# jhbastek/PhysicsInformedDiffusionModels

Hardware: AMD Instinct MI355X
Metric: training samples/sec (UNet+PDE-residual step), 64x64 Darcy (higher is better)
Workload: dtype f32

## Files before the change

### physicsinformeddiffusionmodels_amd/csrc/k_attn_proj.hip

```cpp
#include "pidm_launch.h"

namespace pidm {

static const int kLapDH = 32;
constexpr int kLapSmallNT = 1024;
static const int kLapTileLd = 33;

__device__ __forceinline__ float lap_exp(float x) { return __expf(x); }
__device__ __forceinline__ int lap_row(int r, int half) { return (r & 3) + 8 * (r >> 2) + 4 * half; }

static int lap_nper_div() {
  const char* e = knob("PIDM_LAP_NPER_DIV");
  const int v = e ? atoi(e) : 1;
  return (v == 2 || v == 4) ? v : 1;
}
static int lap_nper(int N, int C, int slabs) {
  int n = (slabs == 1 ? 512 : 256) * 32 / C;
  if (slabs == 3) n = (C == 32) ? 32 : n / 2;
  if (slabs == 2 && n / lap_nper_div() >= 64) n /= lap_nper_div();
  while (n > 32 && N % n) n >>= 1;
  return n;
}

template <int CB>
__global__ void __launch_bounds__(512) lap_kctx_kernel(const float* __restrict__ xn, const float* __restrict__ wqkv,
                                                       float* __restrict__ part, int N, int heads, int nper) {
  constexpr int C = 32 * CB, CP = C + 4;
  HIP_DYNAMIC_SHARED(float, smem)
  float* xs = smem;
  float* fs = smem + (size_t)nper * CP;
  const int tid = threadIdx.x, lane = tid & 63, half = lane >> 5, l31 = lane & 31;
  const int wave = __builtin_amdgcn_readfirstlane(tid >> 6);
  const int NS = N / nper;
  const int b = blockIdx.x / NS, ns = blockIdx.x % NS;
  const int HD = heads * kLapDH;
  const float* xb = xn + ((size_t)b * N + (size_t)ns * nper) * C;
  for (int e = tid; e < nper * (C / 4); e += 512) {
    const int px = e / (C / 4), q = e - px * (C / 4);
    *reinterpret_cast<f32x4*>(xs + (size_t)px * CP + 4 * q) = *reinterpret_cast<const f32x4*>(xb + (size_t)px * C + 4 * q);
  }
  __syncthreads();
  const int h = wave;
  if (h >= heads) return;
  f32x4 wk[C / 8];
  const float* wrow = wqkv + ((size_t)HD + h * kLapDH + l31) * C + 4 * half;
#pragma unroll
  for (int g8 = 0; g8 < C / 8; ++g8) wk[g8] = *reinterpret_cast<const f32x4*>(wrow + 8 * g8);
  f32x16 M[CB];
#pragma unroll
  for (int cb = 0; cb < CB; ++cb)
    for (int r = 0; r < 16; ++r) M[cb][r] = 0.f;
  float mrun = -3.0e38f, zp = 0.f;
  float* fw = fs + wave * 32;
  for (int t = 0; t < nper / 32; ++t) {
    f32x16 kt;
    for (int r = 0; r < 16; ++r) kt[r] = 0.f;
    const float* arow = xs + (size_t)(t * 32 + l31) * CP + 4 * half;
#pragma unroll
    for (int g8 = 0; g8 < C / 8; ++g8) {
      const f32x4 a4 = *reinterpret_cast<const f32x4*>(arow + 8 * g8);
#pragma unroll
      for (int s = 0; s < 4; ++s) kt = __builtin_amdgcn_mfma_f32_32x32x2f32(a4[s], wk[g8][s], kt, 0, 0, 0);
    }
    float tm = kt[0];
#pragma unroll
    for (int r = 1; r < 16; ++r) tm = fmaxf(tm, kt[r]);
    tm = fmaxf(tm, pidm_other_half(tm));
    if (__any(tm > mrun)) {
      const float mn = fmaxf(mrun, tm);
      const float f = lap_exp(mrun - mn);
      zp *= f;
      mrun = mn;
      if (half == 0) fw[l31] = f;
      PIDM_WAVE_LDS_SYNC();
#pragma unroll
      for (int q4 = 0; q4 < 4; ++q4) {
        const f32x4 f4 = *reinterpret_cast<const f32x4*>(fw + 8 * q4 + 4 * half);
#pragma unroll
        for (int cb = 0; cb < CB; ++cb)
#pragma unroll
          for (int i = 0; i < 4; ++i) M[cb][4 * q4 + i] *= f4[i];
      }
      PIDM_WAVE_LDS_SYNC();
    }
#pragma unroll
    for (int r = 0; r < 16; ++r) {
      kt[r] = lap_exp(kt[r] - mrun);
      zp += kt[r];
    }
#pragma unroll
    for (int r = 0; r < 16; ++r) {
      const float* brow = xs + (size_t)(t * 32 + lap_row(r, half)) * CP + l31;
#pragma unroll
      for (int cb = 0; cb < CB; ++cb) M[cb] = __builtin_amdgcn_mfma_f32_32x32x2f32(kt[r], brow[32 * cb], M[cb], 0, 0, 0);
    }
  }
  const float z = zp + pidm_other_half(zp);
  float* o = part + ((size_t)blockIdx.x * heads + h) * (size_t)(32 * C + 64);
#pragma unroll
  for (int cb = 0; cb < CB; ++cb)
#pragma unroll
    for (int r = 0; r < 16; ++r) o[(size_t)lap_row(r, half) * C + 32 * cb + l31] = M[cb][r];
  if (half == 0) {
    o[32 * C + l31] = mrun;
    o[32 * C + 32 + l31] = z;
  }
}

static int lap_nper_split(int N, int C) {
  int n = 256 * 32 / C;
  if (n / lap_nper_div() >= 64) n /= lap_nper_div();
  while (n > 32 && N % n) n >>= 1;
  return n;
}
static int lap_groups(int heads, int ntiles) {
  const char* e = knob("PIDM_LAP_GROUPS");
  int g = 8 / heads;
  if (e && atoi(e) > 0 && atoi(e) < g) g = atoi(e);
  while (g > 1 && ntiles % g) --g;
  return g < 1 ? 1 : g;
}
template <int CB>
__global__ void __launch_bounds__(512) lap_kctx_split_kernel(const float* __restrict__ xn, const float* __restrict__ wqkv,
                                                             float* __restrict__ part, int N, int heads, int nper) {
  constexpr int C = 32 * CB, RA = 6 * C + 16;
  HIP_DYNAMIC_SHARED(float, smemf)
  char* smem = reinterpret_cast<char*>(smemf);
  const int RT = nper * 2 + 16;
  char* XA = smem;
  char* XT = smem + (size_t)nper * RA;
  float* fs = reinterpret_cast<float*>(XT + (size_t)3 * C * RT);
  const int tid = threadIdx.x, lane = tid & 63, half = lane >> 5, l31 = lane & 31;
  const int wave = __builtin_amdgcn_readfirstlane(tid >> 6);
  const int NS = N / nper;
  const int b = blockIdx.x / NS, ns = blockIdx.x % NS;
  const int HD = heads * kLapDH;
  const float* xb = xn + ((size_t)b * N + (size_t)ns * nper) * C;
  {
    constexpr int QN = C / 4, GP = 16 / QN;
    const int q = lane & (QN - 1), pb = (lane & 15) / QN, la = lane >> 4;
    for (int sl = wave; sl < nper / (4 * GP); sl += 8) {
      const int px = (sl * GP + pb) * 4 + la;
      const f32x4 v = *reinterpret_cast<const f32x4*>(xb + (size_t)px * C + 4 * q);
      typedef unsigned u32x2_t __attribute__((ext_vector_type(2)));
      unsigned a0, a1, a2, b0, b1, b2;
      pidm_split3_pk(v[0], v[1], a0, a1, a2);
      pidm_split3_pk(v[2], v[3], b0, b1, b2);
      char* da = XA + (size_t)px * RA + 8 * q;
      *reinterpret_cast<u32x2_t*>(da) = u32x2_t{a0, b0};
      *reinterpret_cast<u32x2_t*>(da + 2 * C) = u32x2_t{a1, b1};
      *reinterpret_cast<u32x2_t*>(da + 4 * C) = u32x2_t{a2, b2};
      unsigned t0 = __float_as_uint(v[0]), t1 = __float_as_uint(v[1]), t2 = __float_as_uint(v[2]), t3 = __float_as_uint(v[3]);
      {
        const auto s02 = __builtin_amdgcn_permlane32_swap(t0, t2, false, false);
        const auto s13 = __builtin_amdgcn_permlane32_swap(t1, t3, false, false);
        const auto s01 = __builtin_amdgcn_permlane16_swap(s02[0], s13[0], false, false);
        const auto s23 = __builtin_amdgcn_permlane16_swap(s02[1], s13[1], false, false);
        t0 = s01[0]; t1 = s01[1]; t2 = s23[0]; t3 = s23[1];
      }
      pidm_split3_pk(__uint_as_float(t0), __uint_as_float(t1), a0, a1, a2);
      pidm_split3_pk(__uint_as_float(t2), __uint_as_float(t3), b0, b1, b2);
      char* dt = XT + (size_t)(4 * q + la) * RT + (size_t)((sl * GP + pb) * 4) * 2;
      *reinterpret_cast<u32x2_t*>(dt) = u32x2_t{a0, b0};
      *reinterpret_cast<u32x2_t*>(dt + (size_t)C * RT) = u32x2_t{a1, b1};
      *reinterpret_cast<u32x2_t*>(dt + (size_t)2 * C * RT) = u32x2_t{a2, b2};
    }
  }
  __syncthreads();
  const int h = wave;
  if (h >= heads) return;
  u32x4 wk[C / 16][3];
  {
    const float* wrow = wqkv + ((size_t)HD + h * kLapDH + l31) * C + 8 * half;
#pragma unroll
    for (int s = 0; s < C / 16; ++s) {
      const f32x4 w0 = *reinterpret_cast<const f32x4*>(wrow + 16 * s), w1 = *reinterpret_cast<const f32x4*>(wrow + 16 * s + 4);
      unsigned p0[4], p1[4], p2[4];
      pidm_split3_pk(w0[0], w0[1], p0[0], p1[0], p2[0]);
      pidm_split3_pk(w0[2], w0[3], p0[1], p1[1], p2[1]);
      pidm_split3_pk(w1[0], w1[1], p0[2], p1[2], p2[2]);
      pidm_split3_pk(w1[2], w1[3], p0[3], p1[3], p2[3]);
      wk[s][0] = u32x4{p0[0], p0[1], p0[2], p0[3]};
      wk[s][1] = u32x4{p1[0], p1[1], p1[2], p1[3]};
      wk[s][2] = u32x4{p2[0], p2[1], p2[2], p2[3]};
    }
  }
  f32x16 M[CB];
#pragma unroll
  for (int cb = 0; cb < CB; ++cb)
    for (int r = 0; r < 16; ++r) M[cb][r] = 0.f;
  float mrun = -3.0e38f, zp = 0.f;
  float* fw = fs + wave * 32;
#define PIDM_LAP_SIX(acc_, a_, b_)                                                                                 \
  acc_ = pidm_mfma_bf16_32x32x16(a_[2], b_[0], acc_);                                                              \
  acc_ = pidm_mfma_bf16_32x32x16(a_[0], b_[2], acc_);                                                              \
  acc_ = pidm_mfma_bf16_32x32x16(a_[1], b_[1], acc_);                                                              \
  acc_ = pidm_mfma_bf16_32x32x16(a_[1], b_[0], acc_);                                                              \
  acc_ = pidm_mfma_bf16_32x32x16(a_[0], b_[1], acc_);                                                              \
  acc_ = pidm_mfma_bf16_32x32x16(a_[0], b_[0], acc_);
  for (int t = 0; t < nper / 32; ++t) {
    f32x16 kt;
    for (int r = 0; r < 16; ++r) kt[r] = 0.f;
    const char* arow = XA + (size_t)(t * 32 + l31) * RA + 16 * half;
#pragma unroll
    for (int s = 0; s < C / 16; ++s) {
      u32x4 xa[3];
#pragma unroll
      for (int pc = 0; pc < 3; ++pc) xa[pc] = *reinterpret_cast<const u32x4*>(arow + pc * 2 * C + 32 * s);
      PIDM_LAP_SIX(kt, xa, wk[s])
    }
    float tm = kt[0];
#pragma unroll
    for (int r = 1; r < 16; ++r) tm = fmaxf(tm, kt[r]);
    tm = fmaxf(tm, pidm_other_half(tm));
    if (__any(tm > mrun)) {
      const float mn = fmaxf(mrun, tm);
      const float f = lap_exp(mrun - mn);
      zp *= f;
      mrun = mn;
      if (half == 0) fw[l31] = f;
      PIDM_WAVE_LDS_SYNC();
#pragma unroll
      for (int q4 = 0; q4 < 4; ++q4) {
        const f32x4 f4 = *reinterpret_cast<const f32x4*>(fw + 8 * q4 + 4 * half);
#pragma unroll
        for (int cb = 0; cb < CB; ++cb)
#pragma unroll
          for (int i = 0; i < 4; ++i) M[cb][4 * q4 + i] *= f4[i];
      }
      PIDM_WAVE_LDS_SYNC();
    }
#pragma unroll
    for (int r = 0; r < 16; ++r) {
      kt[r] = lap_exp(kt[r] - mrun);
      zp += kt[r];
    }
#pragma unroll
    for (int s = 0; s < 2; ++s) {
      u32x4 ea[3];
      {
        unsigned p0[4], p1[4], p2[4];
#pragma unroll
        for (int j = 0; j < 4; ++j) pidm_split3_pk(kt[8 * s + 2 * j], kt[8 * s + 2 * j + 1], p0[j], p1[j], p2[j]);
        ea[0] = u32x4{p0[0], p0[1], p0[2], p0[3]};
        ea[1] = u32x4{p1[0], p1[1], p1[2], p1[3]};
        ea[2] = u32x4{p2[0], p2[1], p2[2], p2[3]};
      }
#pragma unroll
      for (int cb = 0; cb < CB; ++cb) {
        u32x4 xb4[3];
        const char* brow = XT + (size_t)(32 * cb + l31) * RT + (size_t)(t * 32 + 16 * s + 4 * half) * 2;
#pragma unroll
        for (int pc = 0; pc < 3; ++pc) {
          typedef unsigned u32x2_t __attribute__((ext_vector_type(2)));
          const u32x2_t lo = *reinterpret_cast<const u32x2_t*>(brow + (size_t)pc * C * RT);
          const u32x2_t hi = *reinterpret_cast<const u32x2_t*>(brow + (size_t)pc * C * RT + 16);
          xb4[pc] = u32x4{lo[0], lo[1], hi[0], hi[1]};
        }
        PIDM_LAP_SIX(M[cb], ea, xb4)
      }
    }
  }
#undef PIDM_LAP_SIX
  const float z = zp + pidm_other_half(zp);
  float* o = part + ((size_t)blockIdx.x * heads + h) * (size_t)(32 * C + 64);
#pragma unroll
  for (int cb = 0; cb < CB; ++cb)
#pragma unroll
    for (int r = 0; r < 16; ++r) o[(size_t)lap_row(r, half) * C + 32 * cb + l31] = M[cb][r];
  if (half == 0) {
    o[32 * C + l31] = mrun;
    o[32 * C + 32 + l31] = z;
  }
}

__global__ void __launch_bounds__(kLapSmallNT) lap_kctx_final_kernel(const float* __restrict__ part, const float* __restrict__ wqkv,
                                                             const float* __restrict__ wout, float* __restrict__ kst,
                                                             float* __restrict__ Mmat, float* __restrict__ ctx,
                                                             float* __restrict__ P, int N, int heads, int C, int NS) {
  HIP_DYNAMIC_SHARED(float, smem)
  float* sM = smem;
  float* sW = sM + 32 * C;
  float* sC = sW + 32 * (C + 1) + C;
  float* sw = sC + 32 * 33;
  float* sst = sw + NS * 32;
  __shared__ float sm_[32], siz[32];
  constexpr int NT = kLapSmallNT;
  const int b = blockIdx.x / heads, h = blockIdx.x % heads, tid = threadIdx.x;
  const int HD = heads * kLapDH;
  const size_t pstride = (size_t)(32 * C + 64);
  const float* p0 = part + ((size_t)b * NS * heads + h) * pstride;
  for (int e = tid; e < NS * 64; e += NT) sst[e] = p0[(size_t)(e >> 6) * heads * pstride + 32 * C + (e & 63)];
  __syncthreads();
  if (tid < 32) {
    float m = -3.0e38f;
    for (int k = 0; k < NS; ++k) m = fmaxf(m, sst[k * 64 + tid]);
    float z = 0.f;
    for (int k = 0; k < NS; ++k) {
      const float w = lap_exp(sst[k * 64 + tid] - m);
      sw[k * 32 + tid] = w;
      z += sst[k * 64 + 32 + tid] * w;
    }
    sm_[tid] = m;
    siz[tid] = 1.f / z;
    kst[((size_t)blockIdx.x * 32 + tid) * 2] = m;
    kst[((size_t)blockIdx.x * 32 + tid) * 2 + 1] = 1.f / z;
  }
  __syncthreads();
  for (int e = tid; e < 32 * C; e += NT) {
    const int d = e / C;
    float v = 0.f;
    for (int k = 0; k < NS; ++k) v += p0[(size_t)k * heads * pstride + e] * sw[k * 32 + d];
    v *= siz[d];
    sM[e] = v;
    Mmat[(size_t)blockIdx.x * 32 * C + e] = v;
    const int c = e - d * C;
    sW[d * (C + 1) + c] = wqkv[((size_t)2 * HD + h * kLapDH + d) * C + c];
  }
  __syncthreads();
  const float invN = 1.f / (float)N;
  for (int e = tid; e < 1024; e += NT) {
    const int d = e >> 5, ee = e & 31;
    float v = 0.f;
    for (int c = 0; c < C; ++c) v = fmaf(sM[d * C + c], sW[ee * (C + 1) + c], v);
    v *= invN;
    sC[d * 33 + ee] = v;
    ctx[(size_t)blockIdx.x * 1024 + e] = v;
  }
  __syncthreads();
  for (int e = tid; e < 32 * C; e += NT) {
    const int cc = e >> 5, ee = e & 31;
    sW[cc * 33 + ee] = wout[(size_t)cc * HD + h * kLapDH + ee];
  }
  __syncthreads();
  for (int e = tid; e < 32 * C; e += NT) {
    const int d = e / C, cc = e - d * C;
    float v = 0.f;
#pragma unroll
    for (int ee = 0; ee < 32; ++ee) v = fmaf(sC[d * 33 + ee], sW[cc * 33 + ee], v);
    P[(size_t)blockIdx.x * 32 * C + e] = v;
  }
}

template <int CB>
__global__ void __launch_bounds__(256) lap_out_kernel(const float* __restrict__ xn, const float* __restrict__ wqkv,
                                                      const float* __restrict__ P, const float* __restrict__ bias,
                                                      const float* __restrict__ resid, float* __restrict__ y,
                                                      float* __restrict__ qstat, int N, int heads, int tiles_per_wg, float scale) {
  constexpr int C = 32 * CB, CP = C + 4;
  HIP_DYNAMIC_SHARED(float, smem)
  const int HD = heads * kLapDH;
  float* sWq = smem;
  float* sP = smem + (size_t)HD * CP;
  const int tid = threadIdx.x, lane = tid & 63, half = lane >> 5, l31 = lane & 31;
  const int wave = __builtin_amdgcn_readfirstlane(tid >> 6);
  const int wgs_per_img = (N / 32 + tiles_per_wg - 1) / tiles_per_wg;
  const int b = blockIdx.x / wgs_per_img, wg = blockIdx.x % wgs_per_img;
  for (int e = tid; e < HD * (C / 4); e += 256) {
    const int row = e / (C / 4), q = e - row * (C / 4);
    *reinterpret_cast<f32x4*>(sWq + (size_t)row * CP + 4 * q) = *reinterpret_cast<const f32x4*>(wqkv + (size_t)row * C + 4 * q);
    *reinterpret_cast<f32x4*>(sP + (size_t)row * C + 4 * q) = *reinterpret_cast<const f32x4*>(P + ((size_t)b * HD + row) * C + 4 * q);
  }
  __syncthreads();
  const int t_end = (wg + 1) * tiles_per_wg < N / 32 ? (wg + 1) * tiles_per_wg : N / 32;
  for (int t = wg * tiles_per_wg + wave; t < t_end; t += 4) {
    const size_t pix = (size_t)b * N + (size_t)t * 32 + l31;
    f32x4 xt[C / 8];
#pragma unroll
    for (int g8 = 0; g8 < C / 8; ++g8) xt[g8] = *reinterpret_cast<const f32x4*>(xn + pix * C + 8 * g8 + 4 * half);
    f32x16 yacc[CB];
#pragma unroll
    for (int cb = 0; cb < CB; ++cb)
      for (int r = 0; r < 16; ++r) yacc[cb][r] = 0.f;
    for (int h = 0; h < heads; ++h) {
      f32x16 qt;
      for (int r = 0; r < 16; ++r) qt[r] = 0.f;
      const float* wrow = sWq + (size_t)(h * kLapDH + l31) * CP + 4 * half;
#pragma unroll
      for (int g8 = 0; g8 < C / 8; ++g8) {
        const f32x4 w4 = *reinterpret_cast<const f32x4*>(wrow + 8 * g8);
#pragma unroll
        for (int s = 0; s < 4; ++s) qt = __builtin_amdgcn_mfma_f32_32x32x2f32(w4[s], xt[g8][s], qt, 0, 0, 0);
      }
      float mx = qt[0];
#pragma unroll
      for (int r = 1; r < 16; ++r) mx = fmaxf(mx, qt[r]);
      mx = fmaxf(mx, pidm_other_half(mx));
      float sm = 0.f;
#pragma unroll
      for (int r = 0; r < 16; ++r) {
        qt[r] = lap_exp(qt[r] - mx);
        sm += qt[r];
      }
      sm += pidm_other_half(sm);
      const float inv = 1.f / sm;
      if (half == 0) *reinterpret_cast<float2*>(qstat + (pix * heads + h) * 2) = make_float2(mx, inv);
      const float sc = inv * scale;
      const float* prow = sP + (size_t)(h * kLapDH) * C + l31;
#pragma unroll
      for (int r = 0; r < 16; ++r) {
        const float qv = qt[r] * sc;
        const float* pr = prow + (size_t)lap_row(r, half) * C;
#pragma unroll
        for (int cb = 0; cb < CB; ++cb) yacc[cb] = __builtin_amdgcn_mfma_f32_32x32x2f32(pr[32 * cb], qv, yacc[cb], 0, 0, 0);
      }
    }
#pragma unroll
    for (int cb = 0; cb < CB; ++cb)
#pragma unroll
      for (int q4 = 0; q4 < 4; ++q4) {
        const int c0 = 32 * cb + 8 * q4 + 4 * half;
        const f32x4 bv = *reinterpret_cast<const f32x4*>(bias + c0);
        const f32x4 rv = *reinterpret_cast<const f32x4*>(resid + pix * C + c0);
        f32x4 o;
#pragma unroll
        for (int i = 0; i < 4; ++i) o[i] = yacc[cb][4 * q4 + i] + bv[i] + rv[i];
        *reinterpret_cast<f32x4*>(y + pix * C + c0) = o;
      }
  }
}

__global__ void __launch_bounds__(512) lap_out_split_kernel(const float* __restrict__ xn, const float* __restrict__ wqkv,
                                                            const float* __restrict__ P, const float* __restrict__ bias,
                                                            const float* __restrict__ resid, float* __restrict__ y,
                                                            float* __restrict__ qstat, int N, int heads, int tiles_per_wg, float scale) {
  constexpr int C = 32, RA = 6 * C + 16;
  HIP_DYNAMIC_SHARED(float, smemf)
  char* smem = reinterpret_cast<char*>(smemf);
  const int HD = heads * kLapDH;
  const int RT = HD * 2 + 16;
  char* WA = smem;
  char* PT = smem + (size_t)HD * RA;
  const int tid = threadIdx.x, lane = tid & 63, half = lane >> 5, l31 = lane & 31;
  const int wave = __builtin_amdgcn_readfirstlane(tid >> 6);
  const int wgs_per_img = (N / 32 + tiles_per_wg - 1) / tiles_per_wg;
  const int b = blockIdx.x / wgs_per_img, wg = blockIdx.x % wgs_per_img;
  typedef unsigned u32x2_t __attribute__((ext_vector_type(2)));
  {
    const int q = lane & 7, pb = (lane >> 3) & 1, la = lane >> 4;
    for (int sl = wave; sl < HD / 8; sl += 8) {
      const int d = (sl * 2 + pb) * 4 + la;
      const f32x4 v = *reinterpret_cast<const f32x4*>(wqkv + (size_t)d * C + 4 * q);
      const f32x4 w = *reinterpret_cast<const f32x4*>(P + ((size_t)b * HD + d) * C + 4 * q);
      unsigned a0, a1, a2, b0, b1, b2;
      pidm_split3_pk(v[0], v[1], a0, a1, a2);
      pidm_split3_pk(v[2], v[3], b0, b1, b2);
      char* da = WA + (size_t)d * RA + 8 * q;
      *reinterpret_cast<u32x2_t*>(da) = u32x2_t{a0, b0};
      *reinterpret_cast<u32x2_t*>(da + 2 * C) = u32x2_t{a1, b1};
      *reinterpret_cast<u32x2_t*>(da + 4 * C) = u32x2_t{a2, b2};
      unsigned t0 = __float_as_uint(w[0]), t1 = __float_as_uint(w[1]), t2 = __float_as_uint(w[2]), t3 = __float_as_uint(w[3]);
      {
        const auto s02 = __builtin_amdgcn_permlane32_swap(t0, t2, false, false);
        const auto s13 = __builtin_amdgcn_permlane32_swap(t1, t3, false, false);
        const auto s01 = __builtin_amdgcn_permlane16_swap(s02[0], s13[0], false, false);
        const auto s23 = __builtin_amdgcn_permlane16_swap(s02[1], s13[1], false, false);
        t0 = s01[0]; t1 = s01[1]; t2 = s23[0]; t3 = s23[1];
      }
      pidm_split3_pk(__uint_as_float(t0), __uint_as_float(t1), a0, a1, a2);
      pidm_split3_pk(__uint_as_float(t2), __uint_as_float(t3), b0, b1, b2);
      char* dt = PT + (size_t)(4 * q + la) * RT + (size_t)((sl * 2 + pb) * 4) * 2;
      *reinterpret_cast<u32x2_t*>(dt) = u32x2_t{a0, b0};
      *reinterpret_cast<u32x2_t*>(dt + (size_t)C * RT) = u32x2_t{a1, b1};
      *reinterpret_cast<u32x2_t*>(dt + (size_t)2 * C * RT) = u32x2_t{a2, b2};
    }
  }
  __syncthreads();
#define PIDM_LAP_SIX(acc_, a_, b_)                                                                                 \
  acc_ = pidm_mfma_bf16_32x32x16(a_[2], b_[0], acc_);                                                              \
  acc_ = pidm_mfma_bf16_32x32x16(a_[0], b_[2], acc_);                                                              \
  acc_ = pidm_mfma_bf16_32x32x16(a_[1], b_[1], acc_);                                                              \
  acc_ = pidm_mfma_bf16_32x32x16(a_[1], b_[0], acc_);                                                              \
  acc_ = pidm_mfma_bf16_32x32x16(a_[0], b_[1], acc_);                                                              \
  acc_ = pidm_mfma_bf16_32x32x16(a_[0], b_[0], acc_);
  const int t_end = (wg + 1) * tiles_per_wg < N / 32 ? (wg + 1) * tiles_per_wg : N / 32;
  for (int t = wg * tiles_per_wg + wave; t < t_end; t += 8) {
    const size_t pix = (size_t)b * N + (size_t)t * 32 + l31;
    u32x4 xb[C / 16][3];
#pragma unroll
    for (int s = 0; s < C / 16; ++s) {
      const f32x4 x0 = *reinterpret_cast<const f32x4*>(xn + pix * C + 16 * s + 8 * half);
      const f32x4 x1 = *reinterpret_cast<const f32x4*>(xn + pix * C + 16 * s + 8 * half + 4);
      unsigned p0[4], p1[4], p2[4];
      pidm_split3_pk(x0[0], x0[1], p0[0], p1[0], p2[0]);
      pidm_split3_pk(x0[2], x0[3], p0[1], p1[1], p2[1]);
      pidm_split3_pk(x1[0], x1[1], p0[2], p1[2], p2[2]);
      pidm_split3_pk(x1[2], x1[3], p0[3], p1[3], p2[3]);
      xb[s][0] = u32x4{p0[0], p0[1], p0[2], p0[3]};
      xb[s][1] = u32x4{p1[0], p1[1], p1[2], p1[3]};
      xb[s][2] = u32x4{p2[0], p2[1], p2[2], p2[3]};
    }
    f32x16 yacc;
    for (int r = 0; r < 16; ++r) yacc[r] = 0.f;
    for (int h = 0; h < heads; ++h) {
      f32x16 qt;
      for (int r = 0; r < 16; ++r) qt[r] = 0.f;
      const char* wrow = WA + (size_t)(h * kLapDH + l31) * RA + 16 * half;
#pragma unroll
      for (int s = 0; s < C / 16; ++s) {
        u32x4 wa[3];
#pragma unroll
        for (int pc = 0; pc < 3; ++pc) wa[pc] = *reinterpret_cast<const u32x4*>(wrow + pc * 2 * C + 32 * s);
        PIDM_LAP_SIX(qt, wa, xb[s])
      }
      float mx = qt[0];
#pragma unroll
      for (int r = 1; r < 16; ++r) mx = fmaxf(mx, qt[r]);
      mx = fmaxf(mx, pidm_other_half(mx));
      float sm = 0.f;
#pragma unroll
      for (int r = 0; r < 16; ++r) {
        qt[r] = lap_exp(qt[r] - mx);
        sm += qt[r];
      }
      sm += pidm_other_half(sm);
      const float inv = 1.f / sm;
      if (half == 0) *reinterpret_cast<float2*>(qstat + (pix * heads + h) * 2) = make_float2(mx, inv);
      const float sc = inv * scale;
#pragma unroll
      for (int s = 0; s < 2; ++s) {
        u32x4 qb[3], pa[3];
        {
          unsigned p0[4], p1[4], p2[4];
#pragma unroll
          for (int j = 0; j < 4; ++j) pidm_split3_pk(qt[8 * s + 2 * j] * sc, qt[8 * s + 2 * j + 1] * sc, p0[j], p1[j], p2[j]);
          qb[0] = u32x4{p0[0], p0[1], p0[2], p0[3]};
          qb[1] = u32x4{p1[0], p1[1], p1[2], p1[3]};
          qb[2] = u32x4{p2[0], p2[1], p2[2], p2[3]};
        }
        const char* prow = PT + (size_t)l31 * RT + (size_t)(h * kLapDH + 16 * s + 4 * half) * 2;
#pragma unroll
        for (int pc = 0; pc < 3; ++pc) {
          const u32x2_t lo = *reinterpret_cast<const u32x2_t*>(prow + (size_t)pc * C * RT);
          const u32x2_t hi = *reinterpret_cast<const u32x2_t*>(prow + (size_t)pc * C * RT + 16);
          pa[pc] = u32x4{lo[0], lo[1], hi[0], hi[1]};
        }
        PIDM_LAP_SIX(yacc, pa, qb)
      }
    }
#pragma unroll
    for (int q4 = 0; q4 < 4; ++q4) {
      const int c0 = 8 * q4 + 4 * half;
      const f32x4 bv = *reinterpret_cast<const f32x4*>(bias + c0);
      const f32x4 rv = *reinterpret_cast<const f32x4*>(resid + pix * C + c0);
      f32x4 o;
#pragma unroll
      for (int i = 0; i < 4; ++i) o[i] = yacc[4 * q4 + i] + bv[i] + rv[i];
      *reinterpret_cast<f32x4*>(y + pix * C + c0) = o;
    }
  }
#undef PIDM_LAP_SIX
}

template <int CB>
__global__ void __launch_bounds__(512) lap_g_kernel(const float* __restrict__ xn, const float* __restrict__ dy,
                                                    const float* __restrict__ wqkv, const float* __restrict__ qstat,
                                                    float* __restrict__ part, int N, int heads, int nper, float scale) {
  constexpr int C = 32 * CB, CP = C + 4;
  HIP_DYNAMIC_SHARED(float, smem)
  float* xs = smem;
  float* ys = smem + (size_t)nper * CP;
  const int tid = threadIdx.x, lane = tid & 63, half = lane >> 5, l31 = lane & 31;
  const int wave = __builtin_amdgcn_readfirstlane(tid >> 6);
  const int NS = N / nper;
  const int b = blockIdx.x / NS, ns = blockIdx.x % NS;
  const size_t pix0 = (size_t)b * N + (size_t)ns * nper;
  for (int e = tid; e < nper * (C / 4); e += 512) {
    const int px = e / (C / 4), q = e - px * (C / 4);
    *reinterpret_cast<f32x4*>(xs + (size_t)px * CP + 4 * q) = *reinterpret_cast<const f32x4*>(xn + (pix0 + px) * C + 4 * q);
    *reinterpret_cast<f32x4*>(ys + (size_t)px * CP + 4 * q) = *reinterpret_cast<const f32x4*>(dy + (pix0 + px) * C + 4 * q);
  }
  __syncthreads();
  const int h = wave;
  if (h >= heads) return;
  f32x4 wq[C / 8];
  const float* wrow = wqkv + ((size_t)h * kLapDH + l31) * C + 4 * half;
#pragma unroll
  for (int g8 = 0; g8 < C / 8; ++g8) wq[g8] = *reinterpret_cast<const f32x4*>(wrow + 8 * g8);
  f32x16 G[CB];
#pragma unroll
  for (int cb = 0; cb < CB; ++cb)
    for (int r = 0; r < 16; ++r) G[cb][r] = 0.f;
  for (int t = 0; t < nper / 32; ++t) {
    f32x16 qt;
    for (int r = 0; r < 16; ++r) qt[r] = 0.f;
    const float* arow = xs + (size_t)(t * 32 + l31) * CP + 4 * half;
#pragma unroll
    for (int g8 = 0; g8 < C / 8; ++g8) {
      const f32x4 a4 = *reinterpret_cast<const f32x4*>(arow + 8 * g8);
#pragma unroll
      for (int s = 0; s < 4; ++s) qt = __builtin_amdgcn_mfma_f32_32x32x2f32(a4[s], wq[g8][s], qt, 0, 0, 0);
    }
    const float* st = qstat + ((pix0 + (size_t)t * 32) * heads + h) * 2;
#pragma unroll
    for (int r = 0; r < 16; ++r) {
      const int px = lap_row(r, half);
      const float2 s2 = *reinterpret_cast<const float2*>(st + (size_t)px * heads * 2);
      const float qv = lap_exp(qt[r] - s2.x) * s2.y * scale;
      const float* brow = ys + (size_t)(t * 32 + px) * CP + l31;
#pragma unroll
      for (int cb = 0; cb < CB; ++cb) G[cb] = __builtin_amdgcn_mfma_f32_32x32x2f32(qv, brow[32 * cb], G[cb], 0, 0, 0);
    }
  }
  float* o = part + ((size_t)blockIdx.x * heads + h) * (size_t)(32 * C);
#pragma unroll
  for (int cb = 0; cb < CB; ++cb)
#pragma unroll
    for (int r = 0; r < 16; ++r) o[(size_t)lap_row(r, half) * C + 32 * cb + l31] = G[cb][r];
}

template <int CB>
__global__ void __launch_bounds__(512) lap_g_split_kernel(const float* __restrict__ xn, const float* __restrict__ dy,
                                                          const float* __restrict__ wqkv, const float* __restrict__ qstat,
                                                          float* __restrict__ part, int N, int heads, int nper, float scale) {
  constexpr int C = 32 * CB, RA = 6 * C + 16;
  HIP_DYNAMIC_SHARED(float, smemf)
  char* smem = reinterpret_cast<char*>(smemf);
  const int RT = nper * 2 + 16;
  char* XA = smem;
  char* YT = smem + (size_t)nper * RA;
  const int tid = threadIdx.x, lane = tid & 63, half = lane >> 5, l31 = lane & 31;
  const int wave = __builtin_amdgcn_readfirstlane(tid >> 6);
  const int NS = N / nper;
  const int b = blockIdx.x / NS, ns = blockIdx.x % NS;
  const size_t pix0 = (size_t)b * N + (size_t)ns * nper;
  {
    constexpr int QN = C / 4, GP = 16 / QN;
    const int q = lane & (QN - 1), pb = (lane & 15) / QN, la = lane >> 4;
    typedef unsigned u32x2_t __attribute__((ext_vector_type(2)));
    for (int sl = wave; sl < nper / (4 * GP); sl += 8) {
      const int px = (sl * GP + pb) * 4 + la;
      const f32x4 v = *reinterpret_cast<const f32x4*>(xn + (pix0 + px) * C + 4 * q);
      const f32x4 w = *reinterpret_cast<const f32x4*>(dy + (pix0 + px) * C + 4 * q);
      unsigned a0, a1, a2, b0, b1, b2;
      pidm_split3_pk(v[0], v[1], a0, a1, a2);
      pidm_split3_pk(v[2], v[3], b0, b1, b2);
      char* da = XA + (size_t)px * RA + 8 * q;
      *reinterpret_cast<u32x2_t*>(da) = u32x2_t{a0, b0};
      *reinterpret_cast<u32x2_t*>(da + 2 * C) = u32x2_t{a1, b1};
      *reinterpret_cast<u32x2_t*>(da + 4 * C) = u32x2_t{a2, b2};
      unsigned t0 = __float_as_uint(w[0]), t1 = __float_as_uint(w[1]), t2 = __float_as_uint(w[2]), t3 = __float_as_uint(w[3]);
      {
        const auto s02 = __builtin_amdgcn_permlane32_swap(t0, t2, false, false);
        const auto s13 = __builtin_amdgcn_permlane32_swap(t1, t3, false, false);
        const auto s01 = __builtin_amdgcn_permlane16_swap(s02[0], s13[0], false, false);
        const auto s23 = __builtin_amdgcn_permlane16_swap(s02[1], s13[1], false, false);
        t0 = s01[0]; t1 = s01[1]; t2 = s23[0]; t3 = s23[1];
      }
      pidm_split3_pk(__uint_as_float(t0), __uint_as_float(t1), a0, a1, a2);
      pidm_split3_pk(__uint_as_float(t2), __uint_as_float(t3), b0, b1, b2);
      char* dt = YT + (size_t)(4 * q + la) * RT + (size_t)((sl * GP + pb) * 4) * 2;
      *reinterpret_cast<u32x2_t*>(dt) = u32x2_t{a0, b0};
      *reinterpret_cast<u32x2_t*>(dt + (size_t)C * RT) = u32x2_t{a1, b1};
      *reinterpret_cast<u32x2_t*>(dt + (size_t)2 * C * RT) = u32x2_t{a2, b2};
    }
  }
  __syncthreads();
  const int h = wave;
  if (h >= heads) return;
  u32x4 wq[C / 16][3];
  {
    const float* wrow = wqkv + ((size_t)h * kLapDH + l31) * C + 8 * half;
#pragma unroll
    for (int s = 0; s < C / 16; ++s) {
      const f32x4 w0 = *reinterpret_cast<const f32x4*>(wrow + 16 * s), w1 = *reinterpret_cast<const f32x4*>(wrow + 16 * s + 4);
      unsigned p0[4], p1[4], p2[4];
      pidm_split3_pk(w0[0], w0[1], p0[0], p1[0], p2[0]);
      pidm_split3_pk(w0[2], w0[3], p0[1], p1[1], p2[1]);
      pidm_split3_pk(w1[0], w1[1], p0[2], p1[2], p2[2]);
      pidm_split3_pk(w1[2], w1[3], p0[3], p1[3], p2[3]);
      wq[s][0] = u32x4{p0[0], p0[1], p0[2], p0[3]};
      wq[s][1] = u32x4{p1[0], p1[1], p1[2], p1[3]};
      wq[s][2] = u32x4{p2[0], p2[1], p2[2], p2[3]};
    }
  }
  f32x16 G[CB];
#pragma unroll
  for (int cb = 0; cb < CB; ++cb)
    for (int r = 0; r < 16; ++r) G[cb][r] = 0.f;
#define PIDM_LAP_SIX(acc_, a_, b_)                                                                                 \
  acc_ = pidm_mfma_bf16_32x32x16(a_[2], b_[0], acc_);                                                              \
  acc_ = pidm_mfma_bf16_32x32x16(a_[0], b_[2], acc_);                                                              \
  acc_ = pidm_mfma_bf16_32x32x16(a_[1], b_[1], acc_);                                                              \
  acc_ = pidm_mfma_bf16_32x32x16(a_[1], b_[0], acc_);                                                              \
  acc_ = pidm_mfma_bf16_32x32x16(a_[0], b_[1], acc_);                                                              \
  acc_ = pidm_mfma_bf16_32x32x16(a_[0], b_[0], acc_);
  for (int t = 0; t < nper / 32; ++t) {
    f32x16 qt;
    for (int r = 0; r < 16; ++r) qt[r] = 0.f;
    const char* arow = XA + (size_t)(t * 32 + l31) * RA + 16 * half;
#pragma unroll
    for (int s = 0; s < C / 16; ++s) {
      u32x4 xa[3];
#pragma unroll
      for (int pc = 0; pc < 3; ++pc) xa[pc] = *reinterpret_cast<const u32x4*>(arow + pc * 2 * C + 32 * s);
      PIDM_LAP_SIX(qt, xa, wq[s])
    }
    const float* st = qstat + ((pix0 + (size_t)t * 32) * heads + h) * 2;
#pragma unroll
    for (int r = 0; r < 16; ++r) {
      const float2 s2 = *reinterpret_cast<const float2*>(st + (size_t)lap_row(r, half) * heads * 2);
      qt[r] = lap_exp(qt[r] - s2.x) * s2.y * scale;
    }
#pragma unroll
    for (int s = 0; s < 2; ++s) {
      u32x4 ea[3];
      {
        unsigned p0[4], p1[4], p2[4];
#pragma unroll
        for (int j = 0; j < 4; ++j) pidm_split3_pk(qt[8 * s + 2 * j], qt[8 * s + 2 * j + 1], p0[j], p1[j], p2[j]);
        ea[0] = u32x4{p0[0], p0[1], p0[2], p0[3]};
        ea[1] = u32x4{p1[0], p1[1], p1[2], p1[3]};
        ea[2] = u32x4{p2[0], p2[1], p2[2], p2[3]};
      }
#pragma unroll
      for (int cb = 0; cb < CB; ++cb) {
        u32x4 yb4[3];
        const char* brow = YT + (size_t)(32 * cb + l31) * RT + (size_t)(t * 32 + 16 * s + 4 * half) * 2;
#pragma unroll
        for (int pc = 0; pc < 3; ++pc) {
          typedef unsigned u32x2_t __attribute__((ext_vector_type(2)));
          const u32x2_t lo = *reinterpret_cast<const u32x2_t*>(brow + (size_t)pc * C * RT);
          const u32x2_t hi = *reinterpret_cast<const u32x2_t*>(brow + (size_t)pc * C * RT + 16);
          yb4[pc] = u32x4{lo[0], lo[1], hi[0], hi[1]};
        }
        PIDM_LAP_SIX(G[cb], ea, yb4)
      }
    }
  }
#undef PIDM_LAP_SIX
  float* o = part + ((size_t)blockIdx.x * heads + h) * (size_t)(32 * C);
#pragma unroll
  for (int cb = 0; cb < CB; ++cb)
#pragma unroll
    for (int r = 0; r < 16; ++r) o[(size_t)lap_row(r, half) * C + 32 * cb + l31] = G[cb][r];
}

__global__ void __launch_bounds__(kLapSmallNT) lap_mid_kernel(const float* __restrict__ gpart, const float* __restrict__ wqkv,
                                                      const float* __restrict__ wout, const float* __restrict__ ctx,
                                                      const float* __restrict__ Mmat, float* __restrict__ dMmat,
                                                      float* __restrict__ rowdot, float* __restrict__ dwout_part,
                                                      float* __restrict__ dwv_part, int N, int heads, int C, int NS) {
  HIP_DYNAMIC_SHARED(float, smem)
  float* sG = smem;
  float* sW = sG + 32 * (C + 1);
  float* sD = sW + (C > 33 ? C : 33) * 33 + 32 * (C + 1);
  float* sM = sD + 32 * 33;
  constexpr int NT = kLapSmallNT;
  const int b = blockIdx.x / heads, h = blockIdx.x % heads, tid = threadIdx.x;
  const int HD = heads * kLapDH;
  const float* g0 = gpart + ((size_t)b * NS * heads + h) * (size_t)(32 * C);
  for (int e = tid; e < 32 * C; e += NT) {
    const int d = e / C, c = e - d * C;
    float v = 0.f;
    for (int k0 = 0; k0 < NS; k0 += 8) {
      float t[8];
#pragma unroll
      for (int u = 0; u < 8; ++u) t[u] = g0[(size_t)(k0 + u < NS ? k0 + u : 0) * heads * 32 * C + e];
#pragma unroll
      for (int u = 0; u < 8; ++u) v += (k0 + u < NS) ? t[u] : 0.f;
    }
    sG[d * (C + 1) + c] = v;
    sM[d * (C + 1) + c] = Mmat[(size_t)blockIdx.x * 32 * C + e];
    const int cc = e >> 5, ee = e & 31;
    sW[cc * 33 + ee] = wout[(size_t)cc * HD + h * kLapDH + ee];
  }
  __syncthreads();
  for (int e = tid; e < 1024; e += NT) {
    const int d = e >> 5, ee = e & 31;
    float v = 0.f;
    for (int c = 0; c < C; ++c) v = fmaf(sG[d * (C + 1) + c], sW[c * 33 + ee], v);
    sD[d * 33 + ee] = v;
  }
  for (int e = tid; e < 32 * C; e += NT) {
    const int cc = e >> 5, ee = e & 31;
    float v = 0.f;
#pragma unroll 8
    for (int d = 0; d < 32; ++d) v = fmaf(sG[d * (C + 1) + cc], ctx[(size_t)blockIdx.x * 1024 + d * 32 + ee], v);
    dwout_part[((size_t)b * C + cc) * HD + h * kLapDH + ee] = v;
  }
  __syncthreads();
  for (int e = tid; e < 32 * C; e += NT) {
    const int ee = e / C, c = e - ee * C;
    sW[ee * (C + 1) + c] = wqkv[((size_t)2 * HD + h * kLapDH + ee) * C + c];
  }
  __syncthreads();
  const float invN = 1.f / (float)N;
  for (int e = tid; e < 32 * C; e += NT) {
    const int ee = e / C, c = e - ee * C;
    float v = 0.f;
#pragma unroll 8
    for (int d = 0; d < 32; ++d) v = fmaf(sD[d * 33 + ee], sM[d * (C + 1) + c], v);
    dwv_part[((size_t)b * HD + h * kLapDH + ee) * C + c] = v * invN;
  }
  __syncthreads();
  for (int e = tid; e < 32 * C; e += NT) {
    const int d = e / C, c = e - d * C;
    float v = 0.f;
#pragma unroll 8
    for (int ee = 0; ee < 32; ++ee) v = fmaf(sD[d * 33 + ee], sW[ee * (C + 1) + c], v);
    v *= invN;
    dMmat[(size_t)blockIdx.x * 32 * C + e] = v;
    sG[d * (C + 1) + c] = v * sM[d * (C + 1) + c];
  }
  __syncthreads();
  if (tid < 32) {
    float v = 0.f;
    for (int c = 0; c < C; ++c) v += sG[tid * (C + 1) + c];
    rowdot[(size_t)blockIdx.x * 32 + tid] = v;
  }
}

#ifndef PIDM_LAP_TRACE_BUILD
#define PIDM_LAP_TRACE_BUILD 0
#endif
__device__ unsigned long long g_lap_trace[2 * 8 * 16];
template <int CB, bool SP>
__global__ void __launch_bounds__(512) lap_bwd_kernel(const float* __restrict__ xn, const float* __restrict__ dy,
                                                      const float* __restrict__ wqkv, const float* __restrict__ P,
                                                      const float* __restrict__ kst, const float* __restrict__ dMmat,
                                                      const float* __restrict__ rowdot, float* __restrict__ dxn,
                                                      float* __restrict__ dw_part, int N, int heads, int nper, int nsub,
                                                      float scale, int split_dw, int G) {
  constexpr int C = 32 * CB, CP = C + 4;
  static_assert(!SP || CB == 1, "the split projections keep the head's operand matrices in registers: C = 32 only");
  constexpr int WCP = SP ? C : CP;
  constexpr int PR = 208;
  HIP_DYNAMIC_SHARED(float, smem)
  float* xs = smem;
  float* ys = xs + (SP ? 0 : (size_t)nper * CP);
  constexpr int TSZ = CB * 32 * kLapTileLd;
  float* tiles = ys + (SP ? 0 : (size_t)nper * CP);
  float* cst = tiles + (size_t)8 * TSZ;
  constexpr bool WLDS = (CB == 1);
  float* wl = cst + 8 * 96;
  const int RT = nper * 2 + (WLDS ? 0 : 16);
  const int HD = heads * kLapDH;
  char* XT = reinterpret_cast<char*>(wl + (WLDS ? 3 * HD * WCP : 0));
  char* XP = XT + (size_t)3 * C * RT;
  char* YP = XP + (size_t)nper * PR;
  const int tid = threadIdx.x, lane = tid & 63, half = lane >> 5, l31 = lane & 31;
  const int wave = __builtin_amdgcn_readfirstlane(tid >> 6);
  const int NW = N / (nper * nsub);
  const int b = blockIdx.x / NW, nw = blockIdx.x % NW;
  if (WLDS) {
    for (int e = tid; e < 3 * HD * (C / 4); e += 512) {
      const int m = e / (HD * (C / 4)), rem = e - m * (HD * (C / 4));
      const int row = rem / (C / 4), q = rem - row * (C / 4);
      const float* src = (m < 2) ? wqkv + ((size_t)m * HD + row) * C : dMmat + ((size_t)b * HD + row) * C;
      *reinterpret_cast<f32x4*>(wl + ((size_t)m * HD + row) * WCP + 4 * q) = *reinterpret_cast<const f32x4*>(src + 4 * q);
    }
  }
  const int tg = wave / heads, h = wave - tg * heads;
  const bool act = tg < G;
  float* tw = tiles + (size_t)wave * TSZ;
  float* cw = cst + wave * 96;
  if (act && half == 0) {
    cw[l31] = kst[(((size_t)b * heads + h) * 32 + l31) * 2];
    cw[32 + l31] = kst[(((size_t)b * heads + h) * 32 + l31) * 2 + 1];
    cw[64 + l31] = rowdot[((size_t)b * heads + h) * 32 + l31];
  }
  f32x16 dWq[CB], dWk[CB];
  const size_t bh = (size_t)b * heads + (act ? h : 0);
  const int hrow = (act ? h : 0) * kLapDH + l31;
  const float* wq_p = WLDS ? wl + (size_t)hrow * WCP + 4 * half : wqkv + (size_t)hrow * C + 4 * half;
  const float* wk_p = WLDS ? wl + (size_t)(HD + hrow) * WCP + 4 * half : wqkv + ((size_t)HD + hrow) * C + 4 * half;
  const float* dm_p = WLDS ? wl + (size_t)(2 * HD + hrow) * WCP + 4 * half : dMmat + (bh * 32 + l31) * C + 4 * half;
  const float* pp_p = P + (bh * 32 + l31) * C + 4 * half;
  u32x4 fwq[SP ? C / 16 : 1][3], fwk[SP ? C / 16 : 1][3], fpp[SP ? C / 16 : 1][3], fdm[SP ? C / 16 : 1][3];
  if constexpr (SP) {
    __syncthreads();
#pragma unroll
    for (int ks = 0; ks < C / 16; ++ks) {
      const float* srcs[4] = {wl + (size_t)hrow * WCP + 16 * ks + 8 * half, wl + (size_t)(HD + hrow) * WCP + 16 * ks + 8 * half,
                              P + (bh * 32 + l31) * C + 16 * ks + 8 * half, wl + (size_t)(2 * HD + hrow) * WCP + 16 * ks + 8 * half};
#pragma unroll
      for (int m = 0; m < 4; ++m) {
        const f32x4 v0 = *reinterpret_cast<const f32x4*>(srcs[m]), v1 = *reinterpret_cast<const f32x4*>(srcs[m] + 4);
        unsigned q0[4], q1[4], q2[4];
        pidm_split3_pk(v0[0], v0[1], q0[0], q1[0], q2[0]);
        pidm_split3_pk(v0[2], v0[3], q0[1], q1[1], q2[1]);
        pidm_split3_pk(v1[0], v1[1], q0[2], q1[2], q2[2]);
        pidm_split3_pk(v1[2], v1[3], q0[3], q1[3], q2[3]);
        u32x4(&f)[3] = (m == 0) ? fwq[ks] : (m == 1) ? fwk[ks] : (m == 2) ? fpp[ks] : fdm[ks];
        f[0] = u32x4{q0[0], q0[1], q0[2], q0[3]};
        f[1] = u32x4{q1[0], q1[1], q1[2], q1[3]};
        f[2] = u32x4{q2[0], q2[1], q2[2], q2[3]};
      }
    }
  }
  if (act) {
#pragma unroll
    for (int cb = 0; cb < CB; ++cb)
      for (int r = 0; r < 16; ++r) { dWq[cb][r] = 0.f; dWk[cb][r] = 0.f; }
  }
  const int ldT = WLDS ? WCP : C;
  const int hT = act ? h : 0;
  const float* wqT = WLDS ? wl + (size_t)(hT * kLapDH) * WCP + l31 : wqkv + (size_t)hT * kLapDH * C + l31;
  const float* wkT = WLDS ? wl + (size_t)(HD + hT * kLapDH) * WCP + l31 : wqkv + ((size_t)HD + hT * kLapDH) * C + l31;
  const float* dmT = WLDS ? wl + (size_t)(2 * HD + hT * kLapDH) * WCP + l31 : dMmat + ((size_t)b * heads + hT) * 32 * C + l31;

  const float rscale = 1.f / scale;
#define PIDM_LAP_DW(g_, dW_)                                                                                       \
  if (split_dw) {                                                                                                  \
    _Pragma("unroll") for (int r = 0; r < 16; ++r) tw[lap_row(r, half) * kLapTileLd + l31] = g_[r];                \
    PIDM_WAVE_LDS_SYNC();                                                                                          \
    _Pragma("unroll") for (int s = 0; s < 2; ++s) {                                                                \
      float g0[4], g1[4];                                                                                          \
      _Pragma("unroll") for (int e = 0; e < 4; ++e) {                                                              \
        g0[e] = tw[l31 * kLapTileLd + 16 * s + 8 * half + e];                                                      \
        g1[e] = tw[l31 * kLapTileLd + 16 * s + 8 * half + 4 + e];                                                  \
      }                                                                                                            \
      unsigned p0[4], p1[4], p2[4];                                                                                \
      pidm_split3_pk(g0[0], g0[1], p0[0], p1[0], p2[0]);                                                           \
      pidm_split3_pk(g0[2], g0[3], p0[1], p1[1], p2[1]);                                                           \
      pidm_split3_pk(g1[0], g1[1], p0[2], p1[2], p2[2]);                                                           \
      pidm_split3_pk(g1[2], g1[3], p0[3], p1[3], p2[3]);                                                           \
      u32x4 ga[3] = {u32x4{p0[0], p0[1], p0[2], p0[3]}, u32x4{p1[0], p1[1], p1[2], p1[3]}, u32x4{p2[0], p2[1], p2[2], p2[3]}}; \
      _Pragma("unroll") for (int cb = 0; cb < CB; ++cb) {                                                          \
        u32x4 xb4[3];                                                                                              \
        const char* brow = XT + (size_t)(32 * cb + l31) * RT + (size_t)(t * 32 + 16 * s + 8 * half) * 2;           \
        _Pragma("unroll") for (int pc = 0; pc < 3; ++pc) xb4[pc] = *reinterpret_cast<const u32x4*>(brow + (size_t)pc * C * RT); \
        dW_[cb] = pidm_mfma_bf16_32x32x16(ga[2], xb4[0], dW_[cb]);                                                 \
        dW_[cb] = pidm_mfma_bf16_32x32x16(ga[0], xb4[2], dW_[cb]);                                                 \
        dW_[cb] = pidm_mfma_bf16_32x32x16(ga[1], xb4[1], dW_[cb]);                                                 \
        dW_[cb] = pidm_mfma_bf16_32x32x16(ga[1], xb4[0], dW_[cb]);                                                 \
        dW_[cb] = pidm_mfma_bf16_32x32x16(ga[0], xb4[1], dW_[cb]);                                                 \
        dW_[cb] = pidm_mfma_bf16_32x32x16(ga[0], xb4[0], dW_[cb]);                                                 \
      }                                                                                                            \
    }                                                                                                              \
    PIDM_WAVE_LDS_SYNC();                                                                                          \
  } else {                                                                                                         \
    _Pragma("unroll") for (int r = 0; r < 16; ++r) tw[lap_row(r, half) * kLapTileLd + l31] = g_[r];                \
    PIDM_WAVE_LDS_SYNC();                                                                                          \
    _Pragma("unroll") for (int s = 0; s < 16; ++s) {                                                               \
      const float a = tw[l31 * kLapTileLd + 2 * s + half];                                                         \
      const float* brow = xs + (size_t)(t * 32 + 2 * s + half) * CP + l31;                                         \
      _Pragma("unroll") for (int cb = 0; cb < CB; ++cb) dW_[cb] = __builtin_amdgcn_mfma_f32_32x32x2f32(a, brow[32 * cb], dW_[cb], 0, 0, 0); \
    }                                                                                                              \
    PIDM_WAVE_LDS_SYNC();                                                                                          \
  }
#define PIDM_LAP_SIX(acc_, fa_, fb_)                                                                               \
  acc_ = pidm_mfma_bf16_32x32x16(fa_[2], fb_[0], acc_);                                                            \
  acc_ = pidm_mfma_bf16_32x32x16(fa_[0], fb_[2], acc_);                                                            \
  acc_ = pidm_mfma_bf16_32x32x16(fa_[1], fb_[1], acc_);                                                            \
  acc_ = pidm_mfma_bf16_32x32x16(fa_[1], fb_[0], acc_);                                                            \
  acc_ = pidm_mfma_bf16_32x32x16(fa_[0], fb_[1], acc_);                                                            \
  acc_ = pidm_mfma_bf16_32x32x16(fa_[0], fb_[0], acc_);
  const bool order_flip = (split_dw & 2) != 0;
  if ((split_dw & 8) && wave >= 4) __builtin_amdgcn_s_setprio(1);
#if PIDM_LAP_TRACE_BUILD
  const bool tr_on = (split_dw & 4) && blockIdx.x == 0 && (wave & 3) == 0;
  int tr_round = 0;
#define PIDM_LAP_STAMP(i_)                                                                                         \
  if (tr_on && tr_round < 8) {                                                                                     \
    const unsigned long long c__ = clock64();                                                                      \
    if (lane == 0) g_lap_trace[(wave >> 2) * 128 + 16 * tr_round + (i_)] = c__;                                    \
  }
#define PIDM_LAP_TRACE_ONLY(x_) x_
#else
#define PIDM_LAP_STAMP(i_)
#define PIDM_LAP_TRACE_ONLY(x_)
#endif
  split_dw &= 1;
  const bool k_first = (wave & 4) != 0 && order_flip;
  for (int sub = 0; sub < nsub; ++sub) {
  const size_t pix0 = (size_t)b * N + ((size_t)nw * nsub + sub) * nper;
  for (int e = tid; e < nper * (C / 4); e += 512) {
    const int px = e / (C / 4), q = e - px * (C / 4);
    const f32x4 vx = *reinterpret_cast<const f32x4*>(xn + (pix0 + px) * C + 4 * q);
    const f32x4 vy = *reinterpret_cast<const f32x4*>(dy + (pix0 + px) * C + 4 * q);
    if constexpr (SP) {
      typedef unsigned u32x2_t __attribute__((ext_vector_type(2)));
      const size_t o = (size_t)px * PR + ((q >> 2) * 2 + ((q >> 1) & 1)) * 48 + (q & 1) * 8;
      unsigned a0, a1, a2, b0, b1, b2;
      pidm_split3_pk(vx[0], vx[1], a0, a1, a2);
      pidm_split3_pk(vx[2], vx[3], b0, b1, b2);
      *reinterpret_cast<u32x2_t*>(XP + o) = u32x2_t{a0, b0};
      *reinterpret_cast<u32x2_t*>(XP + o + 16) = u32x2_t{a1, b1};
      *reinterpret_cast<u32x2_t*>(XP + o + 32) = u32x2_t{a2, b2};
      pidm_split3_pk(vy[0], vy[1], a0, a1, a2);
      pidm_split3_pk(vy[2], vy[3], b0, b1, b2);
      *reinterpret_cast<u32x2_t*>(YP + o) = u32x2_t{a0, b0};
      *reinterpret_cast<u32x2_t*>(YP + o + 16) = u32x2_t{a1, b1};
      *reinterpret_cast<u32x2_t*>(YP + o + 32) = u32x2_t{a2, b2};
    } else {
      *reinterpret_cast<f32x4*>(xs + (size_t)px * CP + 4 * q) = vx;
      *reinterpret_cast<f32x4*>(ys + (size_t)px * CP + 4 * q) = vy;
    }
  }
  if (split_dw) {
    constexpr int QN = C / 4, GP = 16 / QN;
    const int q = lane & (QN - 1), pb = (lane & 15) / QN, la = lane >> 4;
    typedef unsigned u32x2_t __attribute__((ext_vector_type(2)));
    for (int sl = wave; sl < nper / (4 * GP); sl += 8) {
      const int px = (sl * GP + pb) * 4 + la;
      const f32x4 w = *reinterpret_cast<const f32x4*>(xn + (pix0 + px) * C + 4 * q);
      unsigned t0 = __float_as_uint(w[0]), t1 = __float_as_uint(w[1]), t2 = __float_as_uint(w[2]), t3 = __float_as_uint(w[3]);
      {
        const auto s02 = __builtin_amdgcn_permlane32_swap(t0, t2, false, false);
        const auto s13 = __builtin_amdgcn_permlane32_swap(t1, t3, false, false);
        const auto s01 = __builtin_amdgcn_permlane16_swap(s02[0], s13[0], false, false);
        const auto s23 = __builtin_amdgcn_permlane16_swap(s02[1], s13[1], false, false);
        t0 = s01[0]; t1 = s01[1]; t2 = s23[0]; t3 = s23[1];
      }
      unsigned a0, a1, a2, b0, b1, b2;
      pidm_split3_pk(__uint_as_float(t0), __uint_as_float(t1), a0, a1, a2);
      pidm_split3_pk(__uint_as_float(t2), __uint_as_float(t3), b0, b1, b2);
      char* dt = XT + (size_t)(4 * q + la) * RT + (size_t)((sl * GP + pb) * 4) * 2;
      *reinterpret_cast<u32x2_t*>(dt) = u32x2_t{a0, b0};
      *reinterpret_cast<u32x2_t*>(dt + (size_t)C * RT) = u32x2_t{a1, b1};
      *reinterpret_cast<u32x2_t*>(dt + (size_t)2 * C * RT) = u32x2_t{a2, b2};
    }
  }
  __syncthreads();
  for (int t0 = 0; t0 < nper / 32; t0 += G) {
    const int t = t0 + tg;
    f32x16 dx[CB];
    PIDM_LAP_STAMP(0)
    PIDM_LAP_TRACE_ONLY(int tr_half = 0;)
    if (act) {
      int z0 = 0;
      if (!WLDS) PIDM_OPAQUE_I32(z0);
#pragma unroll
      for (int cb = 0; cb < CB; ++cb)
        for (int r = 0; r < 16; ++r) dx[cb][r] = 0.f;
      const float* xrow = xs + (size_t)(t * 32 + l31) * CP + 4 * half;
      const float* yrow = ys + (size_t)(t * 32 + l31) * CP + 4 * half;
      const char* xpr = XP + (size_t)(t * 32 + l31) * PR + 48 * half;
      const char* ypr = YP + (size_t)(t * 32 + l31) * PR + 48 * half;
      auto q_part = [&]() __attribute__((always_inline)) {
      f32x16 qt, dq;
      for (int r = 0; r < 16; ++r) { qt[r] = 0.f; dq[r] = 0.f; }
      if constexpr (SP) {
#pragma unroll
        for (int ks = 0; ks < C / 16; ++ks) {
          u32x4 xb[3], yb[3];
#pragma unroll
          for (int pc = 0; pc < 3; ++pc) {
            xb[pc] = *reinterpret_cast<const u32x4*>(xpr + 96 * ks + 16 * pc);
            yb[pc] = *reinterpret_cast<const u32x4*>(ypr + 96 * ks + 16 * pc);
          }
          PIDM_LAP_SIX(qt, fwq[ks], xb)
          PIDM_LAP_SIX(dq, fpp[ks], yb)
        }
      } else {
#pragma unroll 2
      for (int g8 = 0; g8 < C / 8; ++g8) {
        const f32x4 w4 = *reinterpret_cast<const f32x4*>(wq_p + z0 + 8 * g8);
        const f32x4 p4 = *reinterpret_cast<const f32x4*>(pp_p + z0 + 8 * g8);
        const f32x4 x4 = *reinterpret_cast<const f32x4*>(xrow + 8 * g8);
        const f32x4 y4 = *reinterpret_cast<const f32x4*>(yrow + 8 * g8);
#pragma unroll
        for (int s = 0; s < 4; ++s) {
          qt = __builtin_amdgcn_mfma_f32_32x32x2f32(w4[s], x4[s], qt, 0, 0, 0);
          dq = __builtin_amdgcn_mfma_f32_32x32x2f32(p4[s], y4[s], dq, 0, 0, 0);
        }
      }
      }
      float mx = qt[0];
#pragma unroll
      for (int r = 1; r < 16; ++r) mx = fmaxf(mx, qt[r]);
      mx = fmaxf(mx, pidm_other_half(mx));
      float sm = 0.f;
#pragma unroll
      for (int r = 0; r < 16; ++r) {
        qt[r] = lap_exp(qt[r] - mx);
        sm += qt[r];
      }
      sm += pidm_other_half(sm);
      const float sc = scale / sm;
      float jd = 0.f;
#pragma unroll
      for (int r = 0; r < 16; ++r) {
        qt[r] *= sc;
        jd += qt[r] * dq[r];
      }
      jd = (jd + pidm_other_half(jd)) * rscale;
#pragma unroll
      for (int r = 0; r < 16; ++r) dq[r] = qt[r] * (dq[r] - jd);
      PIDM_LAP_STAMP(1 + 3 * tr_half)
      if constexpr (WLDS) {
        float wa[16][CB];
#pragma unroll
        for (int r = 0; r < 16; ++r)
#pragma unroll
          for (int cb = 0; cb < CB; ++cb) wa[r][cb] = (wqT + (size_t)lap_row(r, half) * ldT)[32 * cb];
#pragma unroll
        for (int r = 0; r < 16; ++r)
#pragma unroll
          for (int cb = 0; cb < CB; ++cb) dx[cb] = __builtin_amdgcn_mfma_f32_32x32x2f32(wa[r][cb], dq[r], dx[cb], 0, 0, 0);
      } else {
#pragma unroll
        for (int r = 0; r < 16; ++r) {
          const float* wr = wqT + (size_t)lap_row(r, half) * ldT;
#pragma unroll
          for (int cb = 0; cb < CB; ++cb) dx[cb] = __builtin_amdgcn_mfma_f32_32x32x2f32(wr[32 * cb], dq[r], dx[cb], 0, 0, 0);
        }
      }
      PIDM_LAP_STAMP(2 + 3 * tr_half)
      PIDM_LAP_DW(dq, dWq)
      PIDM_LAP_STAMP(3 + 3 * tr_half)
      PIDM_LAP_TRACE_ONLY(tr_half = 1;)
      };
      auto k_part = [&]() __attribute__((always_inline)) {
      f32x16 kt, dk;
      for (int r = 0; r < 16; ++r) { kt[r] = 0.f; dk[r] = 0.f; }
      if constexpr (SP) {
#pragma unroll
        for (int ks = 0; ks < C / 16; ++ks) {
          u32x4 xb[3];
#pragma unroll
          for (int pc = 0; pc < 3; ++pc) xb[pc] = *reinterpret_cast<const u32x4*>(xpr + 96 * ks + 16 * pc);
          PIDM_LAP_SIX(kt, fwk[ks], xb)
          PIDM_LAP_SIX(dk, fdm[ks], xb)
        }
      } else {
#pragma unroll 2
      for (int g8 = 0; g8 < C / 8; ++g8) {
        const f32x4 w4 = *reinterpret_cast<const f32x4*>(wk_p + z0 + 8 * g8);
        const f32x4 m4 = *reinterpret_cast<const f32x4*>(dm_p + z0 + 8 * g8);
        const f32x4 x4 = *reinterpret_cast<const f32x4*>(xrow + 8 * g8);
#pragma unroll
        for (int s = 0; s < 4; ++s) {
          kt = __builtin_amdgcn_mfma_f32_32x32x2f32(w4[s], x4[s], kt, 0, 0, 0);
          dk = __builtin_amdgcn_mfma_f32_32x32x2f32(m4[s], x4[s], dk, 0, 0, 0);
        }
      }
      }
#pragma unroll
      for (int q4 = 0; q4 < 4; ++q4) {
        const f32x4 mx4 = *reinterpret_cast<const f32x4*>(cw + 8 * q4 + 4 * half);
        const f32x4 iz4 = *reinterpret_cast<const f32x4*>(cw + 32 + 8 * q4 + 4 * half);
        const f32x4 rd4 = *reinterpret_cast<const f32x4*>(cw + 64 + 8 * q4 + 4 * half);
#pragma unroll
        for (int i = 0; i < 4; ++i) {
          const int r = 4 * q4 + i;
          kt[r] = lap_exp(kt[r] - mx4[i]) * iz4[i];
          dk[r] = kt[r] * (dk[r] - rd4[i]);
        }
      }
      PIDM_LAP_STAMP(1 + 3 * tr_half)
      if constexpr (WLDS) {
        float wa[16][CB], ma[16][CB];
#pragma unroll
        for (int r = 0; r < 16; ++r)
#pragma unroll
          for (int cb = 0; cb < CB; ++cb) {
            wa[r][cb] = (wkT + (size_t)lap_row(r, half) * ldT)[32 * cb];
            ma[r][cb] = (dmT + (size_t)lap_row(r, half) * ldT)[32 * cb];
          }
#pragma unroll
        for (int r = 0; r < 16; ++r)
#pragma unroll
          for (int cb = 0; cb < CB; ++cb) {
            dx[cb] = __builtin_amdgcn_mfma_f32_32x32x2f32(wa[r][cb], dk[r], dx[cb], 0, 0, 0);
            dx[cb] = __builtin_amdgcn_mfma_f32_32x32x2f32(ma[r][cb], kt[r], dx[cb], 0, 0, 0);
          }
      } else {
#pragma unroll
        for (int r = 0; r < 16; ++r) {
          const float* wr = wkT + (size_t)lap_row(r, half) * ldT;
          const float* mr = dmT + (size_t)lap_row(r, half) * ldT;
#pragma unroll
          for (int cb = 0; cb < CB; ++cb) {
            dx[cb] = __builtin_amdgcn_mfma_f32_32x32x2f32(wr[32 * cb], dk[r], dx[cb], 0, 0, 0);
            dx[cb] = __builtin_amdgcn_mfma_f32_32x32x2f32(mr[32 * cb], kt[r], dx[cb], 0, 0, 0);
          }
        }
      }
      PIDM_LAP_STAMP(2 + 3 * tr_half)
      PIDM_LAP_DW(dk, dWk)
      PIDM_LAP_STAMP(3 + 3 * tr_half)
      PIDM_LAP_TRACE_ONLY(tr_half = 1;)
      };
      if (k_first) { k_part(); q_part(); } else { q_part(); k_part(); }
#pragma unroll
      for (int cb = 0; cb < CB; ++cb)
#pragma unroll
        for (int r = 0; r < 16; ++r) tw[(cb * 32 + lap_row(r, half)) * kLapTileLd + l31] = dx[cb][r];
    }
    PIDM_LAP_STAMP(7)
    __syncthreads();
    PIDM_LAP_STAMP(8)
    for (int e = tid; e < G * 32 * (C / 4); e += 512) {
      const int px = e / (C / 4), c0 = 4 * (e - px * (C / 4));
      const int gq = px >> 5, p31 = px & 31;
      f32x4 o = {0.f, 0.f, 0.f, 0.f};
      for (int w = gq * heads; w < (gq + 1) * heads; ++w) {
        const float* tp = tiles + (size_t)w * TSZ + (size_t)c0 * kLapTileLd + p31;
#pragma unroll
        for (int i = 0; i < 4; ++i) o[i] += tp[i * kLapTileLd];
      }
      *reinterpret_cast<f32x4*>(dxn + (pix0 + (size_t)t0 * 32 + px) * C + c0) = o;
    }
    PIDM_LAP_STAMP(9)
    __syncthreads();
    PIDM_LAP_STAMP(10)
    PIDM_LAP_TRACE_ONLY(++tr_round;)
  }
  }
#undef PIDM_LAP_STAMP
#undef PIDM_LAP_TRACE_ONLY
  for (int m = 0; m < 2 && G > 1; ++m) {
    if (act && tg > 0) {
#pragma unroll
      for (int cb = 0; cb < CB; ++cb)
#pragma unroll
        for (int r = 0; r < 16; ++r) tw[(cb * 32 + lap_row(r, half)) * kLapTileLd + l31] = m ? dWk[cb][r] : dWq[cb][r];
    }
    __syncthreads();
    if (act && tg == 0) {
      for (int g = 1; g < G; ++g) {
        const float* og = tiles + (size_t)(g * heads + h) * TSZ;
#pragma unroll
        for (int cb = 0; cb < CB; ++cb)
#pragma unroll
          for (int r = 0; r < 16; ++r) {
            const float v = og[(cb * 32 + lap_row(r, half)) * kLapTileLd + l31];
            if (m) dWk[cb][r] += v; else dWq[cb][r] += v;
          }
      }
    }
    __syncthreads();
  }
  if (act && tg == 0) {
    float* oq = dw_part + ((size_t)blockIdx.x * 2 * HD + h * kLapDH) * C;
    float* ok = oq + (size_t)HD * C;
#pragma unroll
    for (int cb = 0; cb < CB; ++cb)
#pragma unroll
      for (int r = 0; r < 16; ++r) {
        oq[(size_t)lap_row(r, half) * C + 32 * cb + l31] = dWq[cb][r];
        ok[(size_t)lap_row(r, half) * C + 32 * cb + l31] = dWk[cb][r];
      }
  }
#undef PIDM_LAP_DW
#undef PIDM_LAP_SIX
}

bool lap_ok(int N, int heads, int C, int Cout) {
  return Cout == C && (C == 32 || C == 64) && N % 32 == 0 && N >= 32 && heads >= 1 && heads <= 8;
}

size_t lap_scratch_floats(int B, int N, int heads, int C) {
  const size_t fw = (size_t)B * (N / lap_nper_split(N, C)) * heads * (32 * C + 64);
  const size_t bw = (size_t)B * (N / lap_nper(N, C, 2)) * heads * 32 * C;
  return (fw > bw ? fw : bw) + 64;
}
size_t lap_saved_floats(int B, int heads, int C) { return (size_t)B * heads * (64 + 32 * C + 1024 + 32 * C); }
static int lap_nsub(int N, int C) {
  const int ns = N / lap_nper(N, C, 3);
  int k = 1;
  while (k < 16 && ns % (2 * k) == 0 && ns / (2 * k) >= 8) k *= 2;
  return k;
}
size_t lap_dw_ranges(int N, int C) { return (size_t)(N / lap_nper(N, C, 3) / lap_nsub(N, C)); }

template <int CB>
static int lap_forward_t(const float* xn, const float* wqkv, const float* wout, const float* bias, const float* resid, float* y,
                         float* saved, float* qstat, int B, int N, int heads, float* scratch, hipStream_t st) {
  constexpr int C = 32 * CB;
  const char* spe = knob("PIDM_LAP_SPLIT");
  const bool split1 = !(spe && !atoi(spe));
  const int nper = split1 ? lap_nper_split(N, C) : lap_nper(N, C, 1), NS = N / nper;
  float* kst = saved;
  float* Mmat = kst + (size_t)B * heads * 64;
  float* ctx = Mmat + (size_t)B * heads * 32 * C;
  float* P = ctx + (size_t)B * heads * 1024;
  const size_t lds1 = ((size_t)nper * (C + 4) + 8 * 32) * sizeof(float);
  static bool attr = false;
  if (!attr) {
    (void)hipFuncSetAttribute(reinterpret_cast<const void*>(&lap_kctx_kernel<CB>), hipFuncAttributeMaxDynamicSharedMemorySize, 160 * 1024 - 256);
    (void)hipFuncSetAttribute(reinterpret_cast<const void*>(&lap_out_kernel<CB>), hipFuncAttributeMaxDynamicSharedMemorySize, 160 * 1024 - 256);
    (void)hipFuncSetAttribute(reinterpret_cast<const void*>(&lap_kctx_final_kernel), hipFuncAttributeMaxDynamicSharedMemorySize, 96 * 1024);
    attr = true;
  }
  if (split1) {
    const size_t ldss = (size_t)nper * (6 * C + 16) + (size_t)3 * C * (nper * 2 + 16) + 8 * 32 * sizeof(float);
    static bool attr_s = false;
    if (!attr_s) {
      (void)hipFuncSetAttribute(reinterpret_cast<const void*>(&lap_kctx_split_kernel<CB>), hipFuncAttributeMaxDynamicSharedMemorySize, 160 * 1024 - 256);
      attr_s = true;
    }
    PIDM_PROF_NAME("lap_kctx_split_kernel");
    hipLaunchKernelGGL(HIP_KERNEL_NAME(lap_kctx_split_kernel<CB>), dim3(B * NS), dim3(512), ldss, st, xn, wqkv, scratch, N, heads, nper);
  } else {
    hipLaunchKernelGGL(HIP_KERNEL_NAME(lap_kctx_kernel<CB>), dim3(B * NS), dim3(512), lds1, st, xn, wqkv, scratch, N, heads, nper);
  }
  PIDM_CHECK_LAUNCH("lap_kctx_kernel");
  const size_t lds2 = ((size_t)32 * C + 32 * (C + 1) + C + 32 * 33 + (size_t)NS * 96 + 64) * sizeof(float);
  hipLaunchKernelGGL(lap_kctx_final_kernel, dim3(B * heads), dim3(kLapSmallNT), lds2, st, scratch, wqkv, wout, kst, Mmat, ctx, P, N, heads, C, NS);
  PIDM_CHECK_LAUNCH("lap_kctx_final_kernel");
  const int HD = heads * kLapDH;
  const size_t lds3 = ((size_t)HD * (C + 4) + (size_t)HD * C) * sizeof(float);
  int tpw = 4;
  while ((long)B * ((N / 32 + tpw - 1) / tpw) > 2048 && tpw < 64) tpw *= 2;
  const int wgs = B * ((N / 32 + tpw - 1) / tpw);
  if (split1 && CB == 1 && HD % 8 == 0) {
    int tp8 = 8;
    while ((long)B * ((N / 32 + tp8 - 1) / tp8) > 1024 && tp8 < 64) tp8 *= 2;
    const int wg8 = B * ((N / 32 + tp8 - 1) / tp8);
    const size_t ldso = (size_t)HD * (6 * C + 16) + (size_t)3 * C * (HD * 2 + 16);
    static bool attr_o = false;
    if (!attr_o) {
      (void)hipFuncSetAttribute(reinterpret_cast<const void*>(&lap_out_split_kernel), hipFuncAttributeMaxDynamicSharedMemorySize, 160 * 1024 - 256);
      attr_o = true;
    }
    PIDM_PROF_NAME("lap_out_split_kernel");
    hipLaunchKernelGGL(lap_out_split_kernel, dim3(wg8), dim3(512), ldso, st, xn, wqkv, P, bias, resid, y, qstat, N, heads, tp8, 0.17677669529663687f);
  } else {
    hipLaunchKernelGGL(HIP_KERNEL_NAME(lap_out_kernel<CB>), dim3(wgs), dim3(256), lds3, st, xn, wqkv, P, bias, resid, y, qstat, N, heads, tpw,
                       0.17677669529663687f);
  }
  PIDM_CHECK_LAUNCH("lap_out_kernel");
  return 0;
}

int launch_lap_forward(const float* xn, const float* wqkv, const float* wout, const float* bias, const float* resid, float* y,
                       float* saved, float* qstat, int C, int B, int N, int heads, float* scratch, hipStream_t st) {
  if (!lap_ok(N, heads, C, C)) return fail("projected linear attention: unsupported shape (N=%d heads=%d C=%d)", N, heads, C);
  if (!bias || !resid) return fail("projected linear attention: bias and residual are required");
  if (C == 32) return lap_forward_t<1>(xn, wqkv, wout, bias, resid, y, saved, qstat, B, N, heads, scratch, st);
  return lap_forward_t<2>(xn, wqkv, wout, bias, resid, y, saved, qstat, B, N, heads, scratch, st);
}

template <int CB>
static int lap_backward_t(const float* xn, const float* dy, const float* wqkv, const float* wout, const float* saved, const float* qstat,
                          float* dxn, float* dwqk_part, float* dwv_part, float* dwout_part, float* tmp, int B, int N, int heads,
                          float* scratch, hipStream_t st) {
  constexpr int C = 32 * CB;
  const float scale = 0.17677669529663687f;
  const float* kst = saved;
  const float* Mmat = kst + (size_t)B * heads * 64;
  const float* ctx = Mmat + (size_t)B * heads * 32 * C;
  const float* P = ctx + (size_t)B * heads * 1024;
  float* dMmat = tmp;
  float* rowdot = tmp + (size_t)B * heads * 32 * C;
  static bool attr = false;
  if (!attr) {
    (void)hipFuncSetAttribute(reinterpret_cast<const void*>(&lap_g_kernel<CB>), hipFuncAttributeMaxDynamicSharedMemorySize, 160 * 1024 - 256);
    (void)hipFuncSetAttribute(reinterpret_cast<const void*>(&lap_bwd_kernel<CB, false>), hipFuncAttributeMaxDynamicSharedMemorySize, 160 * 1024 - 256);
    (void)hipFuncSetAttribute(reinterpret_cast<const void*>(&lap_mid_kernel), hipFuncAttributeMaxDynamicSharedMemorySize, 96 * 1024);
    attr = true;
  }
  const int np2 = lap_nper(N, C, 2), NS2 = N / np2;
  const size_t lds1 = (size_t)2 * np2 * (C + 4) * sizeof(float);
  const char* spe = knob("PIDM_LAP_SPLIT");
  if (!(spe && !atoi(spe))) {
    const size_t ldss = (size_t)np2 * (6 * C + 16) + (size_t)3 * C * (np2 * 2 + 16);
    static bool attr_s = false;
    if (!attr_s) {
      (void)hipFuncSetAttribute(reinterpret_cast<const void*>(&lap_g_split_kernel<CB>), hipFuncAttributeMaxDynamicSharedMemorySize, 160 * 1024 - 256);
      attr_s = true;
    }
    PIDM_PROF_NAME("lap_g_split_kernel");
    hipLaunchKernelGGL(HIP_KERNEL_NAME(lap_g_split_kernel<CB>), dim3(B * NS2), dim3(512), ldss, st, xn, dy, wqkv, qstat, scratch, N, heads, np2, scale);
  } else {
    hipLaunchKernelGGL(HIP_KERNEL_NAME(lap_g_kernel<CB>), dim3(B * NS2), dim3(512), lds1, st, xn, dy, wqkv, qstat, scratch, N, heads, np2, scale);
  }
  PIDM_CHECK_LAUNCH("lap_g_kernel");
  const size_t lds2 = ((size_t)32 * (C + 1) + (size_t)(C > 33 ? C : 33) * 33 + 32 * (C + 1) + 32 * 33 + 32 * (C + 1) + 64) * sizeof(float);
  hipLaunchKernelGGL(lap_mid_kernel, dim3(B * heads), dim3(kLapSmallNT), lds2, st, scratch, wqkv, wout, ctx, Mmat, dMmat, rowdot, dwout_part, dwv_part, N,
                     heads, C, NS2);
  PIDM_CHECK_LAUNCH("lap_mid_kernel");
  const int np3 = lap_nper(N, C, 3), nsub = lap_nsub(N, C), NS3 = N / np3 / nsub;
  int G3 = lap_groups(heads, 2), nslab = np3, nsl = nsub;
  if (G3 > 1 && (np3 / 32) % G3) {
    if (nsub % G3 == 0) { nslab = np3 * G3; nsl = nsub / G3; } else G3 = 1;
  }
  const char* ofe = knob("PIDM_LAP_ORDER_FLIP");
  const int oflip = (ofe && !atoi(ofe)) ? 0 : 2;
  const int split_dw = !(spe && !atoi(spe)) ? 1 : 0;
  const char* pre = knob("PIDM_LAP_PRIO");
  const int trbit = (knob("PIDM_LAP_TRACE") ? 4 : 0) | ((pre && atoi(pre)) ? 8 : 0);
  const char* ppe = knob("PIDM_LAP_SPLIT_PROJ");
  if (CB == 1 && split_dw && !(ppe && !atoi(ppe))) {
    const size_t lds3p = ((size_t)8 * 32 * kLapTileLd + 8 * 96 + (size_t)3 * heads * kLapDH * C) * sizeof(float) + (size_t)3 * C * (nslab * 2) +
                         (size_t)2 * nslab * 208;
    if (lds3p > 160 * 1024 - 256) return fail("lap_bwd: %zu B of LDS", lds3p);
    static bool attr_p = false;
    if (!attr_p) {
      (void)hipFuncSetAttribute(reinterpret_cast<const void*>(&lap_bwd_kernel<1, true>), hipFuncAttributeMaxDynamicSharedMemorySize, 160 * 1024 - 256);
      attr_p = true;
    }
    PIDM_PROF_NAME("lap_bwd_kernel<1, true>");
    hipLaunchKernelGGL(HIP_KERNEL_NAME(lap_bwd_kernel<1, true>), dim3(B * NS3), dim3(512), lds3p, st, xn, dy, wqkv, P, kst, dMmat, rowdot, dxn,
                       dwqk_part, N, heads, nslab, nsl, scale, 1 | oflip | trbit, G3);
    PIDM_CHECK_LAUNCH("lap_bwd_kernel");
    return 0;
  }
  const size_t lds3 = ((size_t)2 * nslab * (C + 4) + (size_t)8 * CB * 32 * kLapTileLd + 8 * 96 + (CB == 1 ? 3 * heads * kLapDH * (C + 4) : 0)) * sizeof(float) +
                      (size_t)3 * C * (nslab * 2 + (CB == 1 ? 0 : 16));
  if (lds3 > 160 * 1024 - 256) return fail("lap_bwd: %zu B of LDS", lds3);
  hipLaunchKernelGGL(HIP_KERNEL_NAME(lap_bwd_kernel<CB, false>), dim3(B * NS3), dim3(512), lds3, st, xn, dy, wqkv, P, kst, dMmat, rowdot, dxn, dwqk_part,
                     N, heads, nslab, nsl, scale, split_dw | oflip | trbit, G3);
  PIDM_CHECK_LAUNCH("lap_bwd_kernel");
  return 0;
}

size_t lap_bwd_tmp_floats(int B, int heads, int C) { return (size_t)B * heads * (32 * C + 32) + 64; }

int launch_lap_backward(const float* xn, const float* dy, const float* wqkv, const float* wout, const float* saved, const float* qstat,
                        float* dxn, float* dwqk_part, float* dwv_part, float* dwout_part, float* tmp, int C, int B, int N, int heads,
                        float* scratch, hipStream_t st) {
  if (!lap_ok(N, heads, C, C)) return fail("projected linear attention: unsupported shape (N=%d heads=%d C=%d)", N, heads, C);
  if (C == 32)
    return lap_backward_t<1>(xn, dy, wqkv, wout, saved, qstat, dxn, dwqk_part, dwv_part, dwout_part, tmp, B, N, heads, scratch, st);
  return lap_backward_t<2>(xn, dy, wqkv, wout, saved, qstat, dxn, dwqk_part, dwv_part, dwout_part, tmp, B, N, heads, scratch, st);
}

}

using namespace pidm;

extern "C" size_t pidm_lap_ws(int B, int N, int heads, int C) {
  const size_t HD = (size_t)heads * kLapDH;
  return (lap_scratch_floats(B, N, heads, C) + lap_bwd_tmp_floats(B, heads, C) + (size_t)B * lap_dw_ranges(N, C) * 2 * HD * C +
          (size_t)B * HD * C * 2 + 256) * sizeof(float);
}
extern "C" size_t pidm_lap_saved_floats(int B, int heads, int C) { return lap_saved_floats(B, heads, C); }

extern "C" int pidm_lap_forward(const float* xn, const float* w_qkv, const float* w_out, const float* bias, const float* resid, float* y,
                                float* saved, float* qstat, int C, int B, int N, int heads, void* workspace, void* stream) {
  if (!xn || !w_qkv || !w_out || !y || !saved || !qstat || !workspace) return fail("lap_forward: null buffer");
  return launch_lap_forward(xn, w_qkv, w_out, bias, resid, y, saved, qstat, C, B, N, heads, reinterpret_cast<float*>(workspace), as_stream(stream));
}

extern "C" int pidm_lap_backward(const float* xn, const float* dy, const float* w_qkv, const float* w_out, const float* saved,
                                 const float* qstat, float* d_xn, float* d_w_qkv, float* d_w_out, int C, int B, int N, int heads,
                                 void* workspace, void* stream) {
  if (!xn || !dy || !w_qkv || !w_out || !saved || !qstat || !d_xn || !d_w_qkv || !d_w_out || !workspace) return fail("lap_backward: null buffer");
  if (!lap_ok(N, heads, C, C)) return fail("projected linear attention: unsupported shape (N=%d heads=%d C=%d)", N, heads, C);
  hipStream_t st = as_stream(stream);
  const int HD = heads * kLapDH;
  float* scratch = reinterpret_cast<float*>(workspace);
  float* tmp = scratch + lap_scratch_floats(B, N, heads, C);
  float* dwqk = tmp + lap_bwd_tmp_floats(B, heads, C);
  const int nr = (int)lap_dw_ranges(N, C);
  float* dwv = dwqk + (size_t)B * nr * 2 * HD * C;
  float* dwo = dwv + (size_t)B * HD * C;
  if (launch_lap_backward(xn, dy, w_qkv, w_out, saved, qstat, d_xn, dwqk, dwv, dwo, tmp, C, B, N, heads, scratch, st)) return -1;
  if (launch_split_reduce(dwqk, d_w_qkv, nullptr, nullptr, B * nr, 2 * HD, C, 1, 2 * HD, C, st)) return -1;
  if (launch_split_reduce(dwv, d_w_qkv + (size_t)2 * HD * C, nullptr, nullptr, B, HD, C, 1, HD, C, st)) return -1;
  return launch_split_reduce(dwo, d_w_out, nullptr, nullptr, B, C, HD, 1, C, HD, st);
}

extern "C" int pidm_debug_lap_trace(unsigned long long* out256) {
  return hipMemcpyFromSymbol(out256, HIP_SYMBOL(pidm::g_lap_trace), sizeof(unsigned long long) * 256) == hipSuccess ? 0 : -1;
}
```

Baseline: 7934.

## Prefetch attention input rows and walk ranges persistently in projected linear attention

```diff
diff --git a/physicsinformeddiffusionmodels_amd/csrc/k_attn_proj.hip b/physicsinformeddiffusionmodels_amd/csrc/k_attn_proj.hip
--- a/physicsinformeddiffusionmodels_amd/csrc/k_attn_proj.hip
+++ b/physicsinformeddiffusionmodels_amd/csrc/k_attn_proj.hip
@@ -120,9 +120,97 @@
   while (g > 1 && ntiles % g) --g;
   return g < 1 ? 1 : g;
 }
-template <int CB>
+constexpr int kLapStagePasses = 4;
+#define PIDM_LAP_PIN(x_) asm volatile("" : "+v"(x_))
+typedef unsigned lap_u32x2 __attribute__((ext_vector_type(2)));
+template <int C>
+__device__ __forceinline__ void lap_stage_row(const f32x4& v, char* da) {
+  unsigned a0, a1, a2, b0, b1, b2;
+  pidm_split3_pk(v[0], v[1], a0, a1, a2);
+  pidm_split3_pk(v[2], v[3], b0, b1, b2);
+  *reinterpret_cast<lap_u32x2*>(da) = lap_u32x2{a0, b0};
+  *reinterpret_cast<lap_u32x2*>(da + 2 * C) = lap_u32x2{a1, b1};
+  *reinterpret_cast<lap_u32x2*>(da + 4 * C) = lap_u32x2{a2, b2};
+}
+__device__ __forceinline__ void lap_stage_col(const f32x4& w, char* dt, size_t ps) {
+  unsigned t0 = __float_as_uint(w[0]), t1 = __float_as_uint(w[1]), t2 = __float_as_uint(w[2]), t3 = __float_as_uint(w[3]);
+  {
+    const auto s02 = __builtin_amdgcn_permlane32_swap(t0, t2, false, false);
+    const auto s13 = __builtin_amdgcn_permlane32_swap(t1, t3, false, false);
+    const auto s01 = __builtin_amdgcn_permlane16_swap(s02[0], s13[0], false, false);
+    const auto s23 = __builtin_amdgcn_permlane16_swap(s02[1], s13[1], false, false);
+    t0 = s01[0]; t1 = s01[1]; t2 = s23[0]; t3 = s23[1];
+  }
+  unsigned a0, a1, a2, b0, b1, b2;
+  pidm_split3_pk(__uint_as_float(t0), __uint_as_float(t1), a0, a1, a2);
+  pidm_split3_pk(__uint_as_float(t2), __uint_as_float(t3), b0, b1, b2);
+  *reinterpret_cast<lap_u32x2*>(dt) = lap_u32x2{a0, b0};
+  *reinterpret_cast<lap_u32x2*>(dt + ps) = lap_u32x2{a1, b1};
+  *reinterpret_cast<lap_u32x2*>(dt + 2 * ps) = lap_u32x2{a2, b2};
+}
+template <int C>
+__device__ __forceinline__ void lap_request_rows(const float* __restrict__ src, f32x4 (&v)[kLapStagePasses], int wave, int lane, int nper) {
+  constexpr int QN = C / 4, GP = 16 / QN;
+  const int q = lane & (QN - 1), pb = (lane & 15) / QN, la = lane >> 4;
+  const int nsl = nper / (4 * GP);
+#pragma unroll
+  for (int i = 0; i < kLapStagePasses; ++i) {
+    const int sl = wave + 8 * i < nsl ? wave + 8 * i : nsl - 1;
+    v[i] = *reinterpret_cast<const f32x4*>(src + (size_t)((sl * GP + pb) * 4 + la) * C + 4 * q);
+  }
+}
+template <int C>
+__device__ __forceinline__ void lap_stage_rows(f32x4 (&va)[kLapStagePasses], f32x4 (&vt)[kLapStagePasses], char* XA, char* XT, int RT, int wave,
+                                               int lane, int nper) {
+  constexpr int QN = C / 4, GP = 16 / QN, RA = 6 * C + 16;
+  const int q = lane & (QN - 1), pb = (lane & 15) / QN, la = lane >> 4;
+  const int nsl = nper / (4 * GP);
+#pragma unroll
+  for (int i = 0; i < kLapStagePasses; ++i) {
+    PIDM_LAP_PIN(va[i]);
+    PIDM_LAP_PIN(vt[i]);
+  }
+#pragma unroll
+  for (int i = 0; i < kLapStagePasses; ++i) {
+    const int sl = wave + 8 * i;
+    if (sl < nsl) {
+      const int g4 = sl * GP + pb;
+      lap_stage_row<C>(va[i], XA + (size_t)(g4 * 4 + la) * RA + 8 * q);
+      lap_stage_col(vt[i], XT + (size_t)(4 * q + la) * RT + (size_t)(g4 * 4) * 2, (size_t)C * RT);
+    }
+  }
+}
+template <int C>
+__device__ __forceinline__ void lap_split_frag(const f32x4 (&raw)[C / 8], u32x4 (&out)[C / 16][3]) {
+#pragma unroll
+  for (int s = 0; s < C / 16; ++s) {
+    const f32x4 w0 = raw[2 * s], w1 = raw[2 * s + 1];
+    unsigned p0[4], p1[4], p2[4];
+    pidm_split3_pk(w0[0], w0[1], p0[0], p1[0], p2[0]);
+    pidm_split3_pk(w0[2], w0[3], p0[1], p1[1], p2[1]);
+    pidm_split3_pk(w1[0], w1[1], p0[2], p1[2], p2[2]);
+    pidm_split3_pk(w1[2], w1[3], p0[3], p1[3], p2[3]);
+    out[s][0] = u32x4{p0[0], p0[1], p0[2], p0[3]};
+    out[s][1] = u32x4{p1[0], p1[1], p1[2], p1[3]};
+    out[s][2] = u32x4{p2[0], p2[1], p2[2], p2[3]};
+  }
+}
+#ifndef PIDM_LAP_TRACE_BUILD
+#define PIDM_LAP_TRACE_BUILD 0
+#endif
+__device__ unsigned long long g_lap_trace[2 * 8 * 16];
+#if PIDM_LAP_TRACE_BUILD
+#define PIDM_LAPS_STAMP(i_)                                                                                        \
+  if (blockIdx.x == 0 && (wave & 3) == 0) {                                                                        \
+    const unsigned long long c__ = clock64();                                                                      \
+    if (lane == 0) g_lap_trace[(wave >> 2) * 128 + (i_)] = c__;                                                    \
+  }
+#else
+#define PIDM_LAPS_STAMP(i_)
+#endif
+template <int CB, bool PF>
 __global__ void __launch_bounds__(512) lap_kctx_split_kernel(const float* __restrict__ xn, const float* __restrict__ wqkv,
-                                                             float* __restrict__ part, int N, int heads, int nper) {
+                                                             float* __restrict__ part, int N, int heads, int nper, int nranges) {
   constexpr int C = 32 * CB, RA = 6 * C + 16;
   HIP_DYNAMIC_SHARED(float, smemf)
   char* smem = reinterpret_cast<char*>(smemf);
@@ -132,11 +220,22 @@
   float* fs = reinterpret_cast<float*>(XT + (size_t)3 * C * RT);
   const int tid = threadIdx.x, lane = tid & 63, half = lane >> 5, l31 = lane & 31;
   const int wave = __builtin_amdgcn_readfirstlane(tid >> 6);
-  const int NS = N / nper;
-  const int b = blockIdx.x / NS, ns = blockIdx.x % NS;
   const int HD = heads * kLapDH;
-  const float* xb = xn + ((size_t)b * N + (size_t)ns * nper) * C;
-  {
+  const float* xb = xn + (size_t)blockIdx.x * nper * C;
+  PIDM_LAPS_STAMP(0)
+  u32x4 wk[C / 16][3];
+  [[maybe_unused]] f32x4 v[kLapStagePasses];
+  if constexpr (PF) {
+    lap_request_rows<C>(xb, v, wave, lane, nper);
+    f32x4 wr[C / 8];
+    const float* wrow = wqkv + ((size_t)HD + (wave < heads ? wave : 0) * kLapDH + l31) * C + 8 * half;
+#pragma unroll
+    for (int g8 = 0; g8 < C / 8; ++g8) wr[g8] = *reinterpret_cast<const f32x4*>(wrow + 16 * (g8 >> 1) + 4 * (g8 & 1));
+#pragma unroll
+    for (int g8 = 0; g8 < C / 8; ++g8) PIDM_LAP_PIN(wr[g8]);
+    lap_stage_rows<C>(v, v, XA, XT, RT, wave, lane, nper);
+    lap_split_frag<C>(wr, wk);
+  } else {
     constexpr int QN = C / 4, GP = 16 / QN;
     const int q = lane & (QN - 1), pb = (lane & 15) / QN, la = lane >> 4;
     for (int sl = wave; sl < nper / (4 * GP); sl += 8) {
@@ -167,10 +266,10 @@
     }
   }
   __syncthreads();
+  PIDM_LAPS_STAMP(1)
   const int h = wave;
-  if (h >= heads) return;
-  u32x4 wk[C / 16][3];
-  {
+  if (!PF && h >= heads) return;
+  if constexpr (!PF) {
     const float* wrow = wqkv + ((size_t)HD + h * kLapDH + l31) * C + 8 * half;
 #pragma unroll
     for (int s = 0; s < C / 16; ++s) {
@@ -185,12 +284,6 @@
       wk[s][2] = u32x4{p2[0], p2[1], p2[2], p2[3]};
     }
   }
-  f32x16 M[CB];
-#pragma unroll
-  for (int cb = 0; cb < CB; ++cb)
-    for (int r = 0; r < 16; ++r) M[cb][r] = 0.f;
-  float mrun = -3.0e38f, zp = 0.f;
-  float* fw = fs + wave * 32;
 #define PIDM_LAP_SIX(acc_, a_, b_)                                                                                 \
   acc_ = pidm_mfma_bf16_32x32x16(a_[2], b_[0], acc_);                                                              \
   acc_ = pidm_mfma_bf16_32x32x16(a_[0], b_[2], acc_);                                                              \
@@ -198,80 +291,104 @@
   acc_ = pidm_mfma_bf16_32x32x16(a_[1], b_[0], acc_);                                                              \
   acc_ = pidm_mfma_bf16_32x32x16(a_[0], b_[1], acc_);                                                              \
   acc_ = pidm_mfma_bf16_32x32x16(a_[0], b_[0], acc_);
-  for (int t = 0; t < nper / 32; ++t) {
-    f32x16 kt;
-    for (int r = 0; r < 16; ++r) kt[r] = 0.f;
-    const char* arow = XA + (size_t)(t * 32 + l31) * RA + 16 * half;
-#pragma unroll
-    for (int s = 0; s < C / 16; ++s) {
-      u32x4 xa[3];
-#pragma unroll
-      for (int pc = 0; pc < 3; ++pc) xa[pc] = *reinterpret_cast<const u32x4*>(arow + pc * 2 * C + 32 * s);
-      PIDM_LAP_SIX(kt, xa, wk[s])
-    }
-    float tm = kt[0];
-#pragma unroll
-    for (int r = 1; r < 16; ++r) tm = fmaxf(tm, kt[r]);
-    tm = fmaxf(tm, pidm_other_half(tm));
-    if (__any(tm > mrun)) {
-      const float mn = fmaxf(mrun, tm);
-      const float f = lap_exp(mrun - mn);
-      zp *= f;
-      mrun = mn;
-      if (half == 0) fw[l31] = f;
-      PIDM_WAVE_LDS_SYNC();
-#pragma unroll
-      for (int q4 = 0; q4 < 4; ++q4) {
-        const f32x4 f4 = *reinterpret_cast<const f32x4*>(fw + 8 * q4 + 4 * half);
-#pragma unroll
-        for (int cb = 0; cb < CB; ++cb)
-#pragma unroll
-          for (int i = 0; i < 4; ++i) M[cb][4 * q4 + i] *= f4[i];
-      }
-      PIDM_WAVE_LDS_SYNC();
-    }
-#pragma unroll
-    for (int r = 0; r < 16; ++r) {
-      kt[r] = lap_exp(kt[r] - mrun);
-      zp += kt[r];
-    }
-#pragma unroll
-    for (int s = 0; s < 2; ++s) {
-      u32x4 ea[3];
-      {
-        unsigned p0[4], p1[4], p2[4];
-#pragma unroll
-        for (int j = 0; j < 4; ++j) pidm_split3_pk(kt[8 * s + 2 * j], kt[8 * s + 2 * j + 1], p0[j], p1[j], p2[j]);
-        ea[0] = u32x4{p0[0], p0[1], p0[2], p0[3]};
-        ea[1] = u32x4{p1[0], p1[1], p1[2], p1[3]};
-        ea[2] = u32x4{p2[0], p2[1], p2[2], p2[3]};
-      }
-#pragma unroll
-      for (int cb = 0; cb < CB; ++cb) {
-        u32x4 xb4[3];
-        const char* brow = XT + (size_t)(32 * cb + l31) * RT + (size_t)(t * 32 + 16 * s + 4 * half) * 2;
-#pragma unroll
-        for (int pc = 0; pc < 3; ++pc) {
-          typedef unsigned u32x2_t __attribute__((ext_vector_type(2)));
-          const u32x2_t lo = *reinterpret_cast<const u32x2_t*>(brow + (size_t)pc * C * RT);
-          const u32x2_t hi = *reinterpret_cast<const u32x2_t*>(brow + (size_t)pc * C * RT + 16);
-          xb4[pc] = u32x4{lo[0], lo[1], hi[0], hi[1]};
+  float* fw = fs + wave * 32;
+  const int nt = h < heads ? nper / 32 : 0;
+  for (int rg = blockIdx.x;;) {
+    const int rn = rg + gridDim.x;
+    const bool more = PF && rn < nranges;
+    if (more) lap_request_rows<C>(xn + (size_t)rn * nper * C, v, wave, lane, nper);
+    f32x16 M[CB];
+#pragma unroll
+    for (int cb = 0; cb < CB; ++cb)
+      for (int r = 0; r < 16; ++r) M[cb][r] = 0.f;
+    float mrun = -3.0e38f, zp = 0.f;
+    PIDM_LAPS_STAMP(2)
+    for (int t = 0; t < nt; ++t) {
+      if (t < 8) { PIDM_LAPS_STAMP(3 + t) }
+      f32x16 kt;
+      for (int r = 0; r < 16; ++r) kt[r] = 0.f;
+      const char* arow = XA + (size_t)(t * 32 + l31) * RA + 16 * half;
+#pragma unroll
+      for (int s = 0; s < C / 16; ++s) {
+        u32x4 xa[3];
+#pragma unroll
+        for (int pc = 0; pc < 3; ++pc) xa[pc] = *reinterpret_cast<const u32x4*>(arow + pc * 2 * C + 32 * s);
+        PIDM_LAP_SIX(kt, xa, wk[s])
+      }
+      float tm = kt[0];
+#pragma unroll
+      for (int r = 1; r < 16; ++r) tm = fmaxf(tm, kt[r]);
+      tm = fmaxf(tm, pidm_other_half(tm));
+      if (__any(tm > mrun)) {
+        const float mn = fmaxf(mrun, tm);
+        const float f = lap_exp(mrun - mn);
+        zp *= f;
+        mrun = mn;
+        if (half == 0) fw[l31] = f;
+        PIDM_WAVE_LDS_SYNC();
+#pragma unroll
+        for (int q4 = 0; q4 < 4; ++q4) {
+          const f32x4 f4 = *reinterpret_cast<const f32x4*>(fw + 8 * q4 + 4 * half);
+#pragma unroll
+          for (int cb = 0; cb < CB; ++cb)
+#pragma unroll
+            for (int i = 0; i < 4; ++i) M[cb][4 * q4 + i] *= f4[i];
         }
-        PIDM_LAP_SIX(M[cb], ea, xb4)
-      }
-    }
+        PIDM_WAVE_LDS_SYNC();
+      }
+#pragma unroll
+      for (int r = 0; r < 16; ++r) {
+        kt[r] = lap_exp(kt[r] - mrun);
+        zp += kt[r];
+      }
+#pragma unroll
+      for (int s = 0; s < 2; ++s) {
+        u32x4 ea[3];
+        {
+          unsigned p0[4], p1[4], p2[4];
+#pragma unroll
+          for (int j = 0; j < 4; ++j) pidm_split3_pk(kt[8 * s + 2 * j], kt[8 * s + 2 * j + 1], p0[j], p1[j], p2[j]);
+          ea[0] = u32x4{p0[0], p0[1], p0[2], p0[3]};
+          ea[1] = u32x4{p1[0], p1[1], p1[2], p1[3]};
+          ea[2] = u32x4{p2[0], p2[1], p2[2], p2[3]};
+        }
+#pragma unroll
+        for (int cb = 0; cb < CB; ++cb) {
+          u32x4 xb4[3];
+          const char* brow = XT + (size_t)(32 * cb + l31) * RT + (size_t)(t * 32 + 16 * s + 4 * half) * 2;
+#pragma unroll
+          for (int pc = 0; pc < 3; ++pc) {
+            typedef unsigned u32x2_t __attribute__((ext_vector_type(2)));
+            const u32x2_t lo = *reinterpret_cast<const u32x2_t*>(brow + (size_t)pc * C * RT);
+            const u32x2_t hi = *reinterpret_cast<const u32x2_t*>(brow + (size_t)pc * C * RT + 16);
+            xb4[pc] = u32x4{lo[0], lo[1], hi[0], hi[1]};
+          }
+          PIDM_LAP_SIX(M[cb], ea, xb4)
+        }
+      }
+    }
+    if (h < heads) {
+      const float z = zp + pidm_other_half(zp);
+      float* o = part + ((size_t)rg * heads + h) * (size_t)(32 * C + 64);
+#pragma unroll
+      for (int cb = 0; cb < CB; ++cb)
+#pragma unroll
+        for (int r = 0; r < 16; ++r) o[(size_t)lap_row(r, half) * C + 32 * cb + l31] = M[cb][r];
+      if (half == 0) {
+        o[32 * C + l31] = mrun;
+        o[32 * C + 32 + l31] = z;
+      }
+    }
+    if (!more) break;
+    __syncthreads();
+    PIDM_LAPS_STAMP(12)
+    lap_stage_rows<C>(v, v, XA, XT, RT, wave, lane, nper);
+    __syncthreads();
+    PIDM_LAPS_STAMP(13)
+    rg = rn;
   }
 #undef PIDM_LAP_SIX
-  const float z = zp + pidm_other_half(zp);
-  float* o = part + ((size_t)blockIdx.x * heads + h) * (size_t)(32 * C + 64);
-#pragma unroll
-  for (int cb = 0; cb < CB; ++cb)
-#pragma unroll
-    for (int r = 0; r < 16; ++r) o[(size_t)lap_row(r, half) * C + 32 * cb + l31] = M[cb][r];
-  if (half == 0) {
-    o[32 * C + l31] = mrun;
-    o[32 * C + 32 + l31] = z;
-  }
+  PIDM_LAPS_STAMP(11)
 }
 
 __global__ void __launch_bounds__(kLapSmallNT) lap_kctx_final_kernel(const float* __restrict__ part, const float* __restrict__ wqkv,
@@ -342,7 +459,7 @@
   }
 }
 
-template <int CB>
+template <int CB, bool PF>
 __global__ void __launch_bounds__(256) lap_out_kernel(const float* __restrict__ xn, const float* __restrict__ wqkv,
                                                       const float* __restrict__ P, const float* __restrict__ bias,
                                                       const float* __restrict__ resid, float* __restrict__ y,
@@ -356,18 +473,62 @@
   const int wave = __builtin_amdgcn_readfirstlane(tid >> 6);
   const int wgs_per_img = (N / 32 + tiles_per_wg - 1) / tiles_per_wg;
   const int b = blockIdx.x / wgs_per_img, wg = blockIdx.x % wgs_per_img;
-  for (int e = tid; e < HD * (C / 4); e += 256) {
-    const int row = e / (C / 4), q = e - row * (C / 4);
-    *reinterpret_cast<f32x4*>(sWq + (size_t)row * CP + 4 * q) = *reinterpret_cast<const f32x4*>(wqkv + (size_t)row * C + 4 * q);
-    *reinterpret_cast<f32x4*>(sP + (size_t)row * C + 4 * q) = *reinterpret_cast<const f32x4*>(P + ((size_t)b * HD + row) * C + 4 * q);
+  const int t_end = (wg + 1) * tiles_per_wg < N / 32 ? (wg + 1) * tiles_per_wg : N / 32;
+  const int t_first = wg * tiles_per_wg + wave;
+  f32x4 xnext[C / 8];
+  if constexpr (PF) {
+    const size_t pix = (size_t)b * N + (size_t)(t_first < t_end ? t_first : t_end - 1) * 32 + l31;
+#pragma unroll
+    for (int g8 = 0; g8 < C / 8; ++g8) xnext[g8] = *reinterpret_cast<const f32x4*>(xn + pix * C + 8 * g8 + 4 * half);
+    const int total = HD * (C / 4);
+    for (int e0 = tid; e0 < total; e0 += 256 * 8) {
+      f32x4 a[8], p[8];
+#pragma unroll
+      for (int i = 0; i < 8; ++i) {
+        const int e = e0 + 256 * i < total ? e0 + 256 * i : total - 1;
+        const int row = e / (C / 4), q = e - row * (C / 4);
+        a[i] = *reinterpret_cast<const f32x4*>(wqkv + (size_t)row * C + 4 * q);
+        p[i] = *reinterpret_cast<const f32x4*>(P + ((size_t)b * HD + row) * C + 4 * q);
+      }
+#pragma unroll
+      for (int i = 0; i < 8; ++i) {
+        PIDM_LAP_PIN(a[i]);
+        PIDM_LAP_PIN(p[i]);
+      }
+#pragma unroll
+      for (int i = 0; i < 8; ++i) {
+        const int e = e0 + 256 * i;
+        if (e < total) {
+          const int row = e / (C / 4), q = e - row * (C / 4);
+          *reinterpret_cast<f32x4*>(sWq + (size_t)row * CP + 4 * q) = a[i];
+          *reinterpret_cast<f32x4*>(sP + (size_t)row * C + 4 * q) = p[i];
+        }
+      }
+    }
+  } else {
+    for (int e = tid; e < HD * (C / 4); e += 256) {
+      const int row = e / (C / 4), q = e - row * (C / 4);
+      *reinterpret_cast<f32x4*>(sWq + (size_t)row * CP + 4 * q) = *reinterpret_cast<const f32x4*>(wqkv + (size_t)row * C + 4 * q);
+      *reinterpret_cast<f32x4*>(sP + (size_t)row * C + 4 * q) = *reinterpret_cast<const f32x4*>(P + ((size_t)b * HD + row) * C + 4 * q);
+    }
   }
   __syncthreads();
-  const int t_end = (wg + 1) * tiles_per_wg < N / 32 ? (wg + 1) * tiles_per_wg : N / 32;
-  for (int t = wg * tiles_per_wg + wave; t < t_end; t += 4) {
+  for (int t = t_first; t < t_end; t += 4) {
     const size_t pix = (size_t)b * N + (size_t)t * 32 + l31;
     f32x4 xt[C / 8];
-#pragma unroll
-    for (int g8 = 0; g8 < C / 8; ++g8) xt[g8] = *reinterpret_cast<const f32x4*>(xn + pix * C + 8 * g8 + 4 * half);
+    f32x4 rv4[CB * 4];
+    if constexpr (PF) {
+#pragma unroll
+      for (int g8 = 0; g8 < C / 8; ++g8) xt[g8] = xnext[g8];
+#pragma unroll
+      for (int j = 0; j < CB * 4; ++j) rv4[j] = *reinterpret_cast<const f32x4*>(resid + pix * C + 8 * j + 4 * half);
+      const size_t pixn = (size_t)b * N + (size_t)(t + 4 < t_end ? t + 4 : t) * 32 + l31;
+#pragma unroll
+      for (int g8 = 0; g8 < C / 8; ++g8) xnext[g8] = *reinterpret_cast<const f32x4*>(xn + pixn * C + 8 * g8 + 4 * half);
+    } else {
+#pragma unroll
+      for (int g8 = 0; g8 < C / 8; ++g8) xt[g8] = *reinterpret_cast<const f32x4*>(xn + pix * C + 8 * g8 + 4 * half);
+    }
     f32x16 yacc[CB];
 #pragma unroll
     for (int cb = 0; cb < CB; ++cb)
@@ -411,7 +572,9 @@
       for (int q4 = 0; q4 < 4; ++q4) {
         const int c0 = 32 * cb + 8 * q4 + 4 * half;
         const f32x4 bv = *reinterpret_cast<const f32x4*>(bias + c0);
-        const f32x4 rv = *reinterpret_cast<const f32x4*>(resid + pix * C + c0);
+        f32x4 rv;
+        if constexpr (PF) rv = rv4[cb * 4 + q4];
+        else rv = *reinterpret_cast<const f32x4*>(resid + pix * C + c0);
         f32x4 o;
 #pragma unroll
         for (int i = 0; i < 4; ++i) o[i] = yacc[cb][4 * q4 + i] + bv[i] + rv[i];
@@ -420,6 +583,7 @@
   }
 }
 
+template <bool PF>
 __global__ void __launch_bounds__(512) lap_out_split_kernel(const float* __restrict__ xn, const float* __restrict__ wqkv,
                                                             const float* __restrict__ P, const float* __restrict__ bias,
                                                             const float* __restrict__ resid, float* __restrict__ y,
@@ -436,7 +600,43 @@
   const int wgs_per_img = (N / 32 + tiles_per_wg - 1) / tiles_per_wg;
   const int b = blockIdx.x / wgs_per_img, wg = blockIdx.x % wgs_per_img;
   typedef unsigned u32x2_t __attribute__((ext_vector_type(2)));
-  {
+  PIDM_LAPS_STAMP(16)
+  const int t_end = (wg + 1) * tiles_per_wg < N / 32 ? (wg + 1) * tiles_per_wg : N / 32;
+  const int t_first = wg * tiles_per_wg + wave;
+  f32x4 xr[C / 8], bv4[4];
+  if constexpr (PF) {
+    const int q = lane & 7, pb = (lane >> 3) & 1, la = lane >> 4;
+    const int nsl = HD / 8;
+    f32x4 v[kLapStagePasses], w[kLapStagePasses];
+#pragma unroll
+    for (int i = 0; i < kLapStagePasses; ++i) {
+      const int sl = wave + 8 * i < nsl ? wave + 8 * i : nsl - 1;
+      const int d = (sl * 2 + pb) * 4 + la;
+      v[i] = *reinterpret_cast<const f32x4*>(wqkv + (size_t)d * C + 4 * q);
+      w[i] = *reinterpret_cast<const f32x4*>(P + ((size_t)b * HD + d) * C + 4 * q);
+    }
+    {
+      const size_t pix = (size_t)b * N + (size_t)(t_first < t_end ? t_first : t_end - 1) * 32 + l31;
+#pragma unroll
+      for (int g8 = 0; g8 < C / 8; ++g8) xr[g8] = *reinterpret_cast<const f32x4*>(xn + pix * C + 16 * (g8 >> 1) + 8 * half + 4 * (g8 & 1));
+    }
+#pragma unroll
+    for (int q4 = 0; q4 < 4; ++q4) bv4[q4] = *reinterpret_cast<const f32x4*>(bias + 8 * q4 + 4 * half);
+#pragma unroll
+    for (int i = 0; i < kLapStagePasses; ++i) {
+      PIDM_LAP_PIN(v[i]);
+      PIDM_LAP_PIN(w[i]);
+    }
+#pragma unroll
+    for (int i = 0; i < kLapStagePasses; ++i) {
+      const int sl = wave + 8 * i;
+      if (sl < nsl) {
+        const int g4 = sl * 2 + pb;
+        lap_stage_row<C>(v[i], WA + (size_t)(g4 * 4 + la) * RA + 8 * q);
+        lap_stage_col(w[i], PT + (size_t)(4 * q + la) * RT + (size_t)(g4 * 4) * 2, (size_t)C * RT);
+      }
+    }
+  } else {
     const int q = lane & 7, pb = (lane >> 3) & 1, la = lane >> 4;
     for (int sl = wave; sl < HD / 8; sl += 8) {
       const int d = (sl * 2 + pb) * 4 + la;
@@ -466,6 +666,7 @@
     }
   }
   __syncthreads();
+  PIDM_LAPS_STAMP(17)
 #define PIDM_LAP_SIX(acc_, a_, b_)                                                                                 \
   acc_ = pidm_mfma_bf16_32x32x16(a_[2], b_[0], acc_);                                                              \
   acc_ = pidm_mfma_bf16_32x32x16(a_[0], b_[2], acc_);                                                              \
@@ -473,14 +674,20 @@
   acc_ = pidm_mfma_bf16_32x32x16(a_[1], b_[0], acc_);                                                              \
   acc_ = pidm_mfma_bf16_32x32x16(a_[0], b_[1], acc_);                                                              \
   acc_ = pidm_mfma_bf16_32x32x16(a_[0], b_[0], acc_);
-  const int t_end = (wg + 1) * tiles_per_wg < N / 32 ? (wg + 1) * tiles_per_wg : N / 32;
-  for (int t = wg * tiles_per_wg + wave; t < t_end; t += 8) {
+  for (int t = t_first; t < t_end; t += 8) {
+    PIDM_LAPS_STAMP(19)
     const size_t pix = (size_t)b * N + (size_t)t * 32 + l31;
     u32x4 xb[C / 16][3];
 #pragma unroll
     for (int s = 0; s < C / 16; ++s) {
-      const f32x4 x0 = *reinterpret_cast<const f32x4*>(xn + pix * C + 16 * s + 8 * half);
-      const f32x4 x1 = *reinterpret_cast<const f32x4*>(xn + pix * C + 16 * s + 8 * half + 4);
+      f32x4 x0, x1;
+      if constexpr (PF) {
+        x0 = xr[2 * s];
+        x1 = xr[2 * s + 1];
+      } else {
+        x0 = *reinterpret_cast<const f32x4*>(xn + pix * C + 16 * s + 8 * half);
+        x1 = *reinterpret_cast<const f32x4*>(xn + pix * C + 16 * s + 8 * half + 4);
+      }
       unsigned p0[4], p1[4], p2[4];
       pidm_split3_pk(x0[0], x0[1], p0[0], p1[0], p2[0]);
       pidm_split3_pk(x0[2], x0[3], p0[1], p1[1], p2[1]);
@@ -490,6 +697,14 @@
       xb[s][1] = u32x4{p1[0], p1[1], p1[2], p1[3]};
       xb[s][2] = u32x4{p2[0], p2[1], p2[2], p2[3]};
     }
+    f32x4 rv4[4];
+    if constexpr (PF) {
+#pragma unroll
+      for (int q4 = 0; q4 < 4; ++q4) rv4[q4] = *reinterpret_cast<const f32x4*>(resid + pix * C + 8 * q4 + 4 * half);
+      const size_t pixn = (size_t)b * N + (size_t)(t + 8 < t_end ? t + 8 : t) * 32 + l31;
+#pragma unroll
+      for (int g8 = 0; g8 < C / 8; ++g8) xr[g8] = *reinterpret_cast<const f32x4*>(xn + pixn * C + 16 * (g8 >> 1) + 8 * half + 4 * (g8 & 1));
+    }
     f32x16 yacc;
     for (int r = 0; r < 16; ++r) yacc[r] = 0.f;
     for (int h = 0; h < heads; ++h) {
@@ -541,14 +756,21 @@
 #pragma unroll
     for (int q4 = 0; q4 < 4; ++q4) {
       const int c0 = 8 * q4 + 4 * half;
-      const f32x4 bv = *reinterpret_cast<const f32x4*>(bias + c0);
-      const f32x4 rv = *reinterpret_cast<const f32x4*>(resid + pix * C + c0);
+      f32x4 bv, rv;
+      if constexpr (PF) {
+        bv = bv4[q4];
+        rv = rv4[q4];
+      } else {
+        bv = *reinterpret_cast<const f32x4*>(bias + c0);
+        rv = *reinterpret_cast<const f32x4*>(resid + pix * C + c0);
+      }
       f32x4 o;
 #pragma unroll
       for (int i = 0; i < 4; ++i) o[i] = yacc[4 * q4 + i] + bv[i] + rv[i];
       *reinterpret_cast<f32x4*>(y + pix * C + c0) = o;
     }
   }
+  PIDM_LAPS_STAMP(27)
 #undef PIDM_LAP_SIX
 }
 
@@ -624,6 +846,7 @@
   const int NS = N / nper;
   const int b = blockIdx.x / NS, ns = blockIdx.x % NS;
   const size_t pix0 = (size_t)b * N + (size_t)ns * nper;
+  PIDM_LAPS_STAMP(32)
   {
     constexpr int QN = C / 4, GP = 16 / QN;
     const int q = lane & (QN - 1), pb = (lane & 15) / QN, la = lane >> 4;
@@ -656,6 +879,7 @@
     }
   }
   __syncthreads();
+  PIDM_LAPS_STAMP(33)
   const int h = wave;
   if (h >= heads) return;
   u32x4 wq[C / 16][3];
@@ -685,7 +909,9 @@
   acc_ = pidm_mfma_bf16_32x32x16(a_[1], b_[0], acc_);                                                              \
   acc_ = pidm_mfma_bf16_32x32x16(a_[0], b_[1], acc_);                                                              \
   acc_ = pidm_mfma_bf16_32x32x16(a_[0], b_[0], acc_);
+  PIDM_LAPS_STAMP(34)
   for (int t = 0; t < nper / 32; ++t) {
+    if (t < 8) { PIDM_LAPS_STAMP(35 + t) }
     f32x16 qt;
     for (int r = 0; r < 16; ++r) qt[r] = 0.f;
     const char* arow = XA + (size_t)(t * 32 + l31) * RA + 16 * half;
@@ -734,6 +960,7 @@
   for (int cb = 0; cb < CB; ++cb)
 #pragma unroll
     for (int r = 0; r < 16; ++r) o[(size_t)lap_row(r, half) * C + 32 * cb + l31] = G[cb][r];
+  PIDM_LAPS_STAMP(43)
 }
 
 __global__ void __launch_bounds__(kLapSmallNT) lap_mid_kernel(const float* __restrict__ gpart, const float* __restrict__ wqkv,
@@ -811,10 +1038,6 @@
   }
 }
 
-#ifndef PIDM_LAP_TRACE_BUILD
-#define PIDM_LAP_TRACE_BUILD 0
-#endif
-__device__ unsigned long long g_lap_trace[2 * 8 * 16];
 template <int CB, bool SP>
 __global__ void __launch_bounds__(512) lap_bwd_kernel(const float* __restrict__ xn, const float* __restrict__ dy,
                                                       const float* __restrict__ wqkv, const float* __restrict__ P,
@@ -1257,12 +1480,45 @@
 }
 size_t lap_dw_ranges(int N, int C) { return (size_t)(N / lap_nper(N, C, 3) / lap_nsub(N, C)); }
 
+static int lap_num_cus() {
+  static int ncu = 0;
+  if (!ncu) {
+#ifdef PIDM_BACKEND_NAME
+    ncu = 256;
+#else
+    int dev = 0, v = 0;
+    ncu = (hipGetDevice(&dev) == hipSuccess && hipDeviceGetAttribute(&v, hipDeviceAttributeMultiprocessorCount, dev) == hipSuccess && v > 0) ? v : 256;
+#endif
+  }
+  return ncu;
+}
+static int lap_walk_wgs(int nranges) {
+  const char* e = knob("PIDM_LAP_WGS");
+  const int g = (e && atoi(e) > 0) ? atoi(e) : lap_num_cus();
+  return g < nranges ? g : nranges;
+}
+static int lap_out_tiles(int B, int ntiles, int waves) {
+  const int ncu = lap_num_cus();
+  int best = waves;
+  long best_cost = 0;
+  for (int passes = 1; passes <= 8 && passes * waves <= 64; passes *= 2) {
+    const long wgs = (long)B * ((ntiles + passes * waves - 1) / (passes * waves));
+    const long cost = ((wgs + ncu - 1) / ncu) * (1 + 3 * passes);
+    if (passes == 1 || cost < best_cost) { best = passes * waves; best_cost = cost; }
+  }
+  return best;
+}
+static bool lap_prefetch() {
+  const char* e = knob("PIDM_LAP_PREFETCH");
+  return !(e && !atoi(e));
+}
 template <int CB>
 static int lap_forward_t(const float* xn, const float* wqkv, const float* wout, const float* bias, const float* resid, float* y,
                          float* saved, float* qstat, int B, int N, int heads, float* scratch, hipStream_t st) {
   constexpr int C = 32 * CB;
   const char* spe = knob("PIDM_LAP_SPLIT");
   const bool split1 = !(spe && !atoi(spe));
+  const bool pf = lap_prefetch();
   const int nper = split1 ? lap_nper_split(N, C) : lap_nper(N, C, 1), NS = N / nper;
   float* kst = saved;
   float* Mmat = kst + (size_t)B * heads * 64;
@@ -1272,7 +1528,8 @@
   static bool attr = false;
   if (!attr) {
     (void)hipFuncSetAttribute(reinterpret_cast<const void*>(&lap_kctx_kernel<CB>), hipFuncAttributeMaxDynamicSharedMemorySize, 160 * 1024 - 256);
-    (void)hipFuncSetAttribute(reinterpret_cast<const void*>(&lap_out_kernel<CB>), hipFuncAttributeMaxDynamicSharedMemorySize, 160 * 1024 - 256);
+    (void)hipFuncSetAttribute(reinterpret_cast<const void*>(&lap_out_kernel<CB, false>), hipFuncAttributeMaxDynamicSharedMemorySize, 160 * 1024 - 256);
+    (void)hipFuncSetAttribute(reinterpret_cast<const void*>(&lap_out_kernel<CB, true>), hipFuncAttributeMaxDynamicSharedMemorySize, 160 * 1024 - 256);
     (void)hipFuncSetAttribute(reinterpret_cast<const void*>(&lap_kctx_final_kernel), hipFuncAttributeMaxDynamicSharedMemorySize, 96 * 1024);
     attr = true;
   }
@@ -1280,11 +1537,16 @@
     const size_t ldss = (size_t)nper * (6 * C + 16) + (size_t)3 * C * (nper * 2 + 16) + 8 * 32 * sizeof(float);
     static bool attr_s = false;
     if (!attr_s) {
-      (void)hipFuncSetAttribute(reinterpret_cast<const void*>(&lap_kctx_split_kernel<CB>), hipFuncAttributeMaxDynamicSharedMemorySize, 160 * 1024 - 256);
+      (void)hipFuncSetAttribute(reinterpret_cast<const void*>(&lap_kctx_split_kernel<CB, false>), hipFuncAttributeMaxDynamicSharedMemorySize, 160 * 1024 - 256);
+      (void)hipFuncSetAttribute(reinterpret_cast<const void*>(&lap_kctx_split_kernel<CB, true>), hipFuncAttributeMaxDynamicSharedMemorySize, 160 * 1024 - 256);
       attr_s = true;
     }
     PIDM_PROF_NAME("lap_kctx_split_kernel");
-    hipLaunchKernelGGL(HIP_KERNEL_NAME(lap_kctx_split_kernel<CB>), dim3(B * NS), dim3(512), ldss, st, xn, wqkv, scratch, N, heads, nper);
+    if (pf && nper * C / 256 <= 8 * kLapStagePasses)
+      hipLaunchKernelGGL(HIP_KERNEL_NAME(lap_kctx_split_kernel<CB, true>), dim3(lap_walk_wgs(B * NS)), dim3(512), ldss, st, xn, wqkv, scratch, N, heads, nper,
+                         B * NS);
+    else
+      hipLaunchKernelGGL(HIP_KERNEL_NAME(lap_kctx_split_kernel<CB, false>), dim3(B * NS), dim3(512), ldss, st, xn, wqkv, scratch, N, heads, nper, B * NS);
   } else {
     hipLaunchKernelGGL(HIP_KERNEL_NAME(lap_kctx_kernel<CB>), dim3(B * NS), dim3(512), lds1, st, xn, wqkv, scratch, N, heads, nper);
   }
@@ -1296,21 +1558,30 @@
   const size_t lds3 = ((size_t)HD * (C + 4) + (size_t)HD * C) * sizeof(float);
   int tpw = 4;
   while ((long)B * ((N / 32 + tpw - 1) / tpw) > 2048 && tpw < 64) tpw *= 2;
+  if (pf) tpw = lap_out_tiles(B, N / 32, 4);
   const int wgs = B * ((N / 32 + tpw - 1) / tpw);
   if (split1 && CB == 1 && HD % 8 == 0) {
     int tp8 = 8;
     while ((long)B * ((N / 32 + tp8 - 1) / tp8) > 1024 && tp8 < 64) tp8 *= 2;
+    if (pf) tp8 = lap_out_tiles(B, N / 32, 8);
     const int wg8 = B * ((N / 32 + tp8 - 1) / tp8);
     const size_t ldso = (size_t)HD * (6 * C + 16) + (size_t)3 * C * (HD * 2 + 16);
     static bool attr_o = false;
     if (!attr_o) {
-      (void)hipFuncSetAttribute(reinterpret_cast<const void*>(&lap_out_split_kernel), hipFuncAttributeMaxDynamicSharedMemorySize, 160 * 1024 - 256);
+      (void)hipFuncSetAttribute(reinterpret_cast<const void*>(&lap_out_split_kernel<false>), hipFuncAttributeMaxDynamicSharedMemorySize, 160 * 1024 - 256);
+      (void)hipFuncSetAttribute(reinterpret_cast<const void*>(&lap_out_split_kernel<true>), hipFuncAttributeMaxDynamicSharedMemorySize, 160 * 1024 - 256);
       attr_o = true;
     }
     PIDM_PROF_NAME("lap_out_split_kernel");
-    hipLaunchKernelGGL(lap_out_split_kernel, dim3(wg8), dim3(512), ldso, st, xn, wqkv, P, bias, resid, y, qstat, N, heads, tp8, 0.17677669529663687f);
+    if (pf && HD / 8 <= 8 * kLapStagePasses)
+      hipLaunchKernelGGL(lap_out_split_kernel<true>, dim3(wg8), dim3(512), ldso, st, xn, wqkv, P, bias, resid, y, qstat, N, heads, tp8, 0.17677669529663687f);
+    else
+      hipLaunchKernelGGL(lap_out_split_kernel<false>, dim3(wg8), dim3(512), ldso, st, xn, wqkv, P, bias, resid, y, qstat, N, heads, tp8, 0.17677669529663687f);
+  } else if (pf) {
+    hipLaunchKernelGGL(HIP_KERNEL_NAME(lap_out_kernel<CB, true>), dim3(wgs), dim3(256), lds3, st, xn, wqkv, P, bias, resid, y, qstat, N, heads, tpw,
+                       0.17677669529663687f);
   } else {
-    hipLaunchKernelGGL(HIP_KERNEL_NAME(lap_out_kernel<CB>), dim3(wgs), dim3(256), lds3, st, xn, wqkv, P, bias, resid, y, qstat, N, heads, tpw,
+    hipLaunchKernelGGL(HIP_KERNEL_NAME(lap_out_kernel<CB, false>), dim3(wgs), dim3(256), lds3, st, xn, wqkv, P, bias, resid, y, qstat, N, heads, tpw,
                        0.17677669529663687f);
   }
   PIDM_CHECK_LAUNCH("lap_out_kernel");
```

Result: no change. 7949, median of 4 (+0.2%).
